# GSByeon/multi-speaker-tacotron-tensorflow

Measured on AMD Instinct MI355X. Metric: mel-frames/sec (batched decode), higher is better.
Workload: dtype f32 storage and accumulation; feed-forward GEMMs as 3-term split-bf16 MFMA (bf16x3), the attention memory layer as 6-term split-bf16 MFMA (operands split three ways: fp32-grade); recurrent / decoder mat-vecs exact fp32

## Files before the change

### multi-speaker-tacotron-tensorflow_amd/csrc/taco_decoder_xcd.h

```cpp
#pragma once
#include "taco_kernels.h"

typedef __attribute__((address_space(1))) unsigned long long dx_gu64;
typedef __attribute__((address_space(1))) unsigned dx_gu32;

#define DX_NT 512
#define DX_NW 8
#define DX_GROUP 32
#define DX_NGROUP 8
#define DX_W 256
#define DX_P2 128
#define DX_P3 64
#define DX_SPIN_LIMIT (1u << 21)
#ifndef DX_POLL_SLEEP
#define DX_POLL_SLEEP 0
#endif
#ifndef DX_FIRST_POLL_DELAY
#define DX_FIRST_POLL_DELAY 5
#endif
#ifndef DX_PRIO_OLD
#define DX_PRIO_OLD 1
#endif
#ifndef DX_POLL_DELAY_B
#define DX_POLL_DELAY_B 5
#endif
#define DX_TRACE_STEPS 8
#define DX_TRACE_SLOTS 16

enum {
  DXR_P2 = 0,
  DXR_AGH = 4,
  DXR_AGX = 12,
  DXR_AC = 18,
  DXR_G1H = 22,
  DXR_G1A = 30,
  DXR_G1B = 46,
  DXR_G1C = 62,
  DXR_G2H = 66,
  DXR_G2X = 74,
  DXR_G2C = 86,
  DXR_P1C = 90,
  DXR_P1O = 94,
  DXR_F = 98,
  DX_NREG = 106
};

enum { DXS_P2 = 0, DXS_HATT = 128, DXS_CTX = 384, DXS_OUT2 = 640, DXS_T = 896, DXS_H1 = 1152, DXS_OUT1 = 1408, DXS_H2 = 1664,
       DXS_LD = 1920 };
enum { DXB_P1 = 0, DXB_P2, DXB_AR, DXB_AU, DXB_AC, DXB_G1R, DXB_G1U, DXB_G1X, DXB_O0, DXB_G1C, DXB_G2R, DXB_G2U, DXB_G2C, DXB_F0, DXB_F1,
       DXB_P3, DXB_N };
enum { DXRB_AR = 0, DXRB_AU, DXRB_AX, DXRB_G1R, DXRB_G1U, DXRB_G1X, DXRB_O0, DXRB_N };

enum { DXT_P1 = 0, DXT_HA, DXT_RA, DXT_UA, DXT_CA, DXT_RHA, DXT_Q, DXT_O0, DXT_R1, DXT_U1, DXT_C1, DXT_RH1, DXT_H1, DXT_O1,
       DXT_R2, DXT_U2, DXT_C2, DXT_RH2, DXT_H2, DXT_O2, DXT_N };

struct DxX { int p1, p2, rha, ha, sc, ctx, rh1, h1, o1, rh2, h2, p3, fb, total; };
__host__ __device__ inline DxX dx_xlayout(int RG, int T_in) {
  DxX x; int o = 0;
  x.p1 = o; o += RG * DX_W;  x.p2 = o; o += RG * DX_P2; x.rha = o; o += RG * DX_W; x.ha = o; o += RG * DX_W;
  x.sc = o; o += DX_GROUP * T_in;
  x.ctx = o; o += RG * DX_W; x.rh1 = o; o += RG * DX_W; x.h1 = o; o += RG * DX_W; x.o1 = o; o += RG * DX_W;
  x.rh2 = o; o += RG * DX_W; x.h2 = o; o += RG * DX_W;
  x.p3 = o; o += RG * DX_P3;
  x.fb = o; o += RG * DX_P2;
  x.total = o;
  return x;
}
__host__ __device__ inline size_t dx_lds_floats(int RG, int T_in, bool teacher = false, int AW = DX_W) {
  const int Pr = DX_GROUP / RG, DC = DX_W / Pr, Tpad = (T_in + 3) & ~3;
  const int Pc = Pr < 8 ? Pr : 8, Pp = Pr / Pc, DS = AW / Pc, TS = (T_in + Pp - 1) / Pp;
  size_t n = 0;
  n += (size_t)RG * DXS_LD;
  n += (size_t)TS * DS;
  n += (size_t)T_in * DC;
  n += 4 * (size_t)Tpad;
  n += 3 * 64;
  n += (size_t)DX_NW * 64;
  n += (size_t)DXB_N * DX_NW;
  n += (size_t)DXRB_N * RG * DX_NW;
  n += (size_t)((T_in + 63) & ~63);
  if (teacher) n += (size_t)RG * DX_W;
  n += 64;
  return n;
}
__host__ __device__ inline int dx_score_blocks(int RG) { const int Pr = DX_GROUP / RG; return Pr < 8 ? Pr : 8; }
__host__ __device__ inline int dx_q_regs(int RG, int AW = DX_W) { return (AW / dx_score_blocks(RG)) / 2; }

struct DxArgs {
  const float* wpack;
  const float* qpack;
  const float* b_p1_0; const float* b_p1c; const float* b_p2;
  const float* b_p3;
  const float* b_ag; const float* b_ac;
  const float* b_g1f;
  const float* b_g1c; const float* b_g2g; const float* b_g2c;
  const float* b_f;
  const float* att_v; const float* att_b; const float* score_bias;
  const float* keys; const float* values;
  const float* h_att0; const float* h10; const float* h20;
  const float* manual;
  const float* rowbias;
  const float* teacher;
  const float* p1o_raw;
  int own_fb;
  float* tape; size_t tstride;
  float* tp_p2; float* tp_ctx; int ld_p2, ld_ctx;
  float* tp_e; float* tp_alpha;
  int mels;
  float* mel; float* hist; int* nz; float* dbg;
  unsigned long long* xbuf; unsigned* ctl; unsigned* err; long long* trace;
  int B, T_in, n, rM, att_type, grp0, ngroups, force_wt, dbgw;
  int trc_member, trc_tid;
};

#define DX_DPP0(v, ctrl) __int_as_float(__builtin_amdgcn_update_dpp(0, __float_as_int(v), (ctrl), 0xF, 0xF, false))
#define DX_DPPZ(v, ctrl, rmask, bmask) __int_as_float(__builtin_amdgcn_update_dpp(0, __float_as_int(v), (ctrl), (rmask), (bmask), true))
__device__ __forceinline__ float dx_allsum(float v) {
  v += DX_DPP0(v, 0xB1);
  v += DX_DPP0(v, 0x4E);
  v += DX_DPP0(v, 0x141);
  v += DX_DPP0(v, 0x140);
  v += DX_DPPZ(v, 0x142, 0xA, 0xF);
  v += DX_DPPZ(v, 0x143, 0xC, 0xF);
  return __int_as_float(__builtin_amdgcn_readlane(__float_as_int(v), 63));
}
__device__ __forceinline__ float dx_allmax(float v) {
  v = fmaxf(v, DX_DPP0(v, 0xB1)); v = fmaxf(v, DX_DPP0(v, 0x4E)); v = fmaxf(v, DX_DPP0(v, 0x141)); v = fmaxf(v, DX_DPP0(v, 0x140));
  const float a = __int_as_float(__builtin_amdgcn_readlane(__float_as_int(v), 0)), b = __int_as_float(__builtin_amdgcn_readlane(__float_as_int(v), 16));
  const float c = __int_as_float(__builtin_amdgcn_readlane(__float_as_int(v), 32)), d = __int_as_float(__builtin_amdgcn_readlane(__float_as_int(v), 48));
  return fmaxf(fmaxf(a, b), fmaxf(c, d));
}
__device__ __forceinline__ float dx_quadsum(float v) { v += DX_DPP0(v, 0xB1); v += DX_DPP0(v, 0x4E); return v; }
__device__ __forceinline__ float dx_scan(float v) {
  float t = v + DX_DPPZ(v, 0x111, 0xF, 0xF);
  t += DX_DPPZ(v, 0x112, 0xF, 0xF);
  t += DX_DPPZ(v, 0x113, 0xF, 0xF);
  t += DX_DPPZ(t, 0x114, 0xF, 0xE);
  t += DX_DPPZ(t, 0x118, 0xF, 0xC);
  t += DX_DPPZ(t, 0x142, 0xA, 0xF);
  t += DX_DPPZ(t, 0x143, 0xC, 0xF);
  return t;
}
__device__ __forceinline__ float dx_sigmoid_fast(float x) { return __builtin_amdgcn_rcpf(1.0f + __builtin_amdgcn_exp2f(-1.4426950408889634f * x)); }

template <int REG0, int NCOLS, int RG, int NW = DX_NREG, int LD = DXS_LD>
__device__ __forceinline__ void dx_pass(const float (&W)[NW], const float* x, int lane, float (&acc)[NCOLS][RG]) {
#pragma unroll
  for (int r = 0; r < RG; ++r) {
    const float4 xv = *reinterpret_cast<const float4*>(x + r * LD + 4 * lane);
#pragma unroll
    for (int c = 0; c < NCOLS; ++c) {
      acc[c][r] = fmaf(W[REG0 + 4 * c + 0], xv.x, acc[c][r]);
      acc[c][r] = fmaf(W[REG0 + 4 * c + 1], xv.y, acc[c][r]);
      acc[c][r] = fmaf(W[REG0 + 4 * c + 2], xv.z, acc[c][r]);
      acc[c][r] = fmaf(W[REG0 + 4 * c + 3], xv.w, acc[c][r]);
    }
  }
}
template <int REG0, int NCOLS, int RG>
__device__ __forceinline__ void dx_pass2(const float (&W)[DX_NREG], const float* x, int lane, float (&acc)[NCOLS][RG]) {
#pragma unroll
  for (int r = 0; r < RG; ++r) {
    const float2 xv = *reinterpret_cast<const float2*>(x + r * DXS_LD + 2 * lane);
#pragma unroll
    for (int c = 0; c < NCOLS; ++c) {
      acc[c][r] = fmaf(W[REG0 + 2 * c + 0], xv.x, acc[c][r]);
      acc[c][r] = fmaf(W[REG0 + 2 * c + 1], xv.y, acc[c][r]);
    }
  }
}
template <int REG0, int NCOLS, int RG>
__device__ __forceinline__ void dx_pass1(const float (&W)[DX_NREG], const float* x, int lane, float (&acc)[NCOLS][RG]) {
#pragma unroll
  for (int r = 0; r < RG; ++r) {
    const float xv = x[r * DXS_LD + lane];
#pragma unroll
    for (int c = 0; c < NCOLS; ++c) acc[c][r] = fmaf(W[REG0 + c], xv, acc[c][r]);
  }
}
template <int NCOLS, int RG>
__device__ __forceinline__ void dx_zero(float (&acc)[NCOLS][RG]) {
#pragma unroll
  for (int c = 0; c < NCOLS; ++c)
#pragma unroll
    for (int r = 0; r < RG; ++r) acc[c][r] = 0.f;
}
template <int RG> struct DxRL { static constexpr int value = RG >= 4 ? RG / 4 : 1; };
template <int RG>
__device__ __forceinline__ int dx_row(int lane, int q) {
  if (RG >= 4) return (lane & 1) * (RG / 2) + ((lane >> 1) & 1) * (RG / 4) + q;
  if (RG == 2) return lane & 1;
  return 0;
}
__device__ __forceinline__ float dx_xrow16(float v) {
  const unsigned u = __float_as_uint(v);
  auto r = __builtin_amdgcn_permlane16_swap(u, u, false, false);
  return __uint_as_float(r[0]) + __uint_as_float(r[1]);
}
__device__ __forceinline__ float dx_xrow32(float v) {
  const unsigned u = __float_as_uint(v);
  auto r = __builtin_amdgcn_permlane32_swap(u, u, false, false);
  return __uint_as_float(r[0]) + __uint_as_float(r[1]);
}
template <int NC, int RG>
__device__ __forceinline__ void dx_reduce(const float (&a)[NC][RG], float (&out)[NC][DxRL<RG>::value], int lane) {
  constexpr int RL = DxRL<RG>::value;
  const bool b0 = (lane & 1) != 0, b1 = (lane & 2) != 0;
  float d[NC][RL];
  if (RG >= 4) {
    constexpr int H = RG / 2, Q = RG / 4;
    float b[NC][H];
#pragma unroll
    for (int c = 0; c < NC; ++c)
#pragma unroll
      for (int p = 0; p < H; ++p) {
        const float keep = b0 ? a[c][H + p] : a[c][p], send = b0 ? a[c][p] : a[c][H + p];
        b[c][p] = keep + DX_DPP0(send, 0xB1);
      }
#pragma unroll
    for (int c = 0; c < NC; ++c)
#pragma unroll
      for (int q = 0; q < Q; ++q) {
        const float keep = b1 ? b[c][Q + q] : b[c][q], send = b1 ? b[c][q] : b[c][Q + q];
        d[c][q] = keep + DX_DPP0(send, 0x4E);
      }
  } else if (RG == 2) {
#pragma unroll
    for (int c = 0; c < NC; ++c) {
      const float keep = b0 ? a[c][1] : a[c][0], send = b0 ? a[c][0] : a[c][1];
      const float t = keep + DX_DPP0(send, 0xB1);
      d[c][0] = t + DX_DPP0(t, 0x4E);
    }
  } else {
#pragma unroll
    for (int c = 0; c < NC; ++c) {
      const float t = a[c][0] + DX_DPP0(a[c][0], 0xB1);
      d[c][0] = t + DX_DPP0(t, 0x4E);
    }
  }
#pragma unroll
  for (int c = 0; c < NC; ++c)
#pragma unroll
    for (int q = 0; q < RL; ++q) d[c][q] += DX_DPP0(d[c][q], 0x124);
#pragma unroll
  for (int c = 0; c < NC; ++c)
#pragma unroll
    for (int q = 0; q < RL; ++q) d[c][q] += DX_DPP0(d[c][q], 0x128);
#pragma unroll
  for (int c = 0; c < NC; ++c)
#pragma unroll
    for (int q = 0; q < RL; ++q) d[c][q] = dx_xrow16(d[c][q]);
#pragma unroll
  for (int c = 0; c < NC; ++c)
#pragma unroll
    for (int q = 0; q < RL; ++q) out[c][q] = dx_xrow32(d[c][q]);
}

#ifndef DX_DIET
#define DX_DIET 1
#endif
#define DX_NWP (DX_NREG / 2)
__host__ __device__ constexpr int dxw_two(int base, int r, int h) { return base + (r - base) / 2 + 4 * h; }
__host__ __device__ constexpr int dxw_src(int k, int h, int PD) {
  const int r = 2 * k;
  if (r >= DXR_AGH && r < DXR_AGX) return dxw_two(DXR_AGH, r, h);
  if (r >= DXR_AGX && r < DXR_AC) return PD == 3 ? r + h : (r < DXR_AGX + 4 ? DXR_AGX + (r - DXR_AGX) / 2 + 2 * h : r + h);
  if (r >= DXR_G1H && r < DXR_G1A) return dxw_two(DXR_G1H, r, h);
  if (r >= DXR_G1A && r < DXR_G1C) return dxw_two(DXR_G1A + 8 * ((r - DXR_G1A) / 8), r, h);
  if (r >= DXR_G2H && r < DXR_G2X) return dxw_two(DXR_G2H, r, h);
  if (r >= DXR_G2X && r < DXR_G2X + 8) return dxw_two(DXR_G2X, r, h);
  if (r >= DXR_F) return dxw_two(DXR_F, r, h);
  return r + h;
}
#define DXQ_FMA(acc, xs, wp) \
  do { if (DX_DIET) acc = __builtin_elementwise_fma((taco_f32x2){xs, xs}, wp, acc); else { acc.x = fmaf((wp).x, xs, acc.x); acc.y = fmaf((wp).y, xs, acc.y); } } while (0)
template <int RG>
__device__ __forceinline__ void dxq_zero(taco_f32x2 (&acc)[RG]) {
#pragma unroll
  for (int r = 0; r < RG; ++r) acc[r] = (taco_f32x2){0.f, 0.f};
}
template <int REG0, int RG, int LD = DXS_LD>
__device__ __forceinline__ void dxw_single(const taco_f32x2 (&WP)[DX_NWP], const float* x, int lane, float (&acc)[1][RG]) {
  constexpr int k = REG0 / 2;
#pragma unroll
  for (int r = 0; r < RG; ++r) {
    const float4 xv = *reinterpret_cast<const float4*>(x + r * LD + 4 * lane);
    acc[0][r] = fmaf(WP[k].x, xv.x, acc[0][r]); acc[0][r] = fmaf(WP[k].y, xv.y, acc[0][r]);
    acc[0][r] = fmaf(WP[k + 1].x, xv.z, acc[0][r]); acc[0][r] = fmaf(WP[k + 1].y, xv.w, acc[0][r]);
  }
}
template <int REG0, int RG, int LD = DXS_LD>
__device__ __forceinline__ void dxw_pair(const taco_f32x2 (&WP)[DX_NWP], const float* x, int lane, taco_f32x2 (&acc)[RG]) {
  constexpr int k = REG0 / 2;
#pragma unroll
  for (int r = 0; r < RG; ++r) {
    const float4 xv = *reinterpret_cast<const float4*>(x + r * LD + 4 * lane);
    DXQ_FMA(acc[r], xv.x, WP[k]); DXQ_FMA(acc[r], xv.y, WP[k + 1]); DXQ_FMA(acc[r], xv.z, WP[k + 2]); DXQ_FMA(acc[r], xv.w, WP[k + 3]);
  }
}
template <int REG0, int RG, int LD = DXS_LD>
__device__ __forceinline__ void dxw_quad(const taco_f32x2 (&WP)[DX_NWP], const float* x, int lane, taco_f32x2 (&p0)[RG], taco_f32x2 (&p1)[RG]) {
  constexpr int k = REG0 / 2;
#pragma unroll
  for (int r = 0; r < RG; ++r) {
    const float4 xv = *reinterpret_cast<const float4*>(x + r * LD + 4 * lane);
    DXQ_FMA(p0[r], xv.x, WP[k]); DXQ_FMA(p1[r], xv.x, WP[k + 4]);
    DXQ_FMA(p0[r], xv.y, WP[k + 1]); DXQ_FMA(p1[r], xv.y, WP[k + 5]);
    DXQ_FMA(p0[r], xv.z, WP[k + 2]); DXQ_FMA(p1[r], xv.z, WP[k + 6]);
    DXQ_FMA(p0[r], xv.w, WP[k + 3]); DXQ_FMA(p1[r], xv.w, WP[k + 7]);
  }
}
template <int REGP, int REGS, int RG, int LD = DXS_LD>
__device__ __forceinline__ void dxw_pair_single(const taco_f32x2 (&WP)[DX_NWP], const float* x, int lane, taco_f32x2 (&p)[RG], float (&sg)[1][RG]) {
  constexpr int k = REGP / 2, ks = REGS / 2;
#pragma unroll
  for (int r = 0; r < RG; ++r) {
    const float4 xv = *reinterpret_cast<const float4*>(x + r * LD + 4 * lane);
    DXQ_FMA(p[r], xv.x, WP[k]); sg[0][r] = fmaf(WP[ks].x, xv.x, sg[0][r]);
    DXQ_FMA(p[r], xv.y, WP[k + 1]); sg[0][r] = fmaf(WP[ks].y, xv.y, sg[0][r]);
    DXQ_FMA(p[r], xv.z, WP[k + 2]); sg[0][r] = fmaf(WP[ks + 1].x, xv.z, sg[0][r]);
    DXQ_FMA(p[r], xv.w, WP[k + 3]); sg[0][r] = fmaf(WP[ks + 1].y, xv.w, sg[0][r]);
  }
}
template <int RG>
__device__ __forceinline__ void dxw_agx2(const taco_f32x2 (&WP)[DX_NWP], const float* x, int lane, taco_f32x2 (&p)[RG], float (&sg)[1][RG]) {
  constexpr int k = DXR_AGX / 2;
#pragma unroll
  for (int r = 0; r < RG; ++r) {
    const float2 xv = *reinterpret_cast<const float2*>(x + r * DXS_LD + 2 * lane);
    DXQ_FMA(p[r], xv.x, WP[k]); sg[0][r] = fmaf(WP[k + 2].x, xv.x, sg[0][r]);
    DXQ_FMA(p[r], xv.y, WP[k + 1]); sg[0][r] = fmaf(WP[k + 2].y, xv.y, sg[0][r]);
  }
}
template <int RG>
__device__ __forceinline__ void dxw_agx1(const taco_f32x2 (&WP)[DX_NWP], const float* x, int lane, taco_f32x2 (&p)[RG], float (&sg)[1][RG]) {
  constexpr int k = DXR_AGX / 2;
#pragma unroll
  for (int r = 0; r < RG; ++r) {
    const float xv = x[r * DXS_LD + lane];
    DXQ_FMA(p[r], xv, WP[k]); sg[0][r] = fmaf(WP[k + 1].x, xv, sg[0][r]);
  }
}
template <int RG>
__device__ __forceinline__ void dxw_p3(const taco_f32x2 (&WP)[DX_NWP], const float* x, int lane, float (&acc)[1][RG]) {
  constexpr int k = DXR_AGX / 2;
#pragma unroll
  for (int r = 0; r < RG; ++r) {
    const float2 xv = *reinterpret_cast<const float2*>(x + r * DXS_LD + 2 * lane);
    acc[0][r] = fmaf(WP[k + 1].y, xv.x, acc[0][r]); acc[0][r] = fmaf(WP[k + 2].x, xv.y, acc[0][r]);
  }
}
template <int RG>
__device__ __forceinline__ int dxs_row(int lane, int q) {
  if (!DX_DIET) return dx_row<RG>(lane & 3, q);
  if (RG >= 8) return ((lane >> 4) & 1) * (RG / 4) + (lane >> 5) * (RG / 2) + q;
  if (RG == 4) return lane >> 4;
  if (RG == 2) return lane >> 5;
  return 0;
}
template <int RG>
__device__ __forceinline__ bool dxs_epl(int lane) {
  if (!DX_DIET) return lane < (RG >= 4 ? 4 : RG);
  return RG >= 4 ? (lane & 15) == 0 : RG == 2 ? (lane & 31) == 0 : lane == 0;
}
template <int NC, int RG>
__device__ __forceinline__ void dxs_reduce(const float (&a)[NC][RG], float (&out)[NC][DxRL<RG>::value], int lane) {
  if constexpr (!DX_DIET) { dx_reduce<NC, RG>(a, out, lane); return; }
  else {
    constexpr int RL = DxRL<RG>::value;
    float d[NC][RL];
    if constexpr (RG >= 4) {
      constexpr int Hh = RG / 2, Q = RG / 4;
      float b[NC][Hh];
#pragma unroll
      for (int c = 0; c < NC; ++c)
#pragma unroll
        for (int p = 0; p < Hh; ++p) {
          auto r = __builtin_amdgcn_permlane32_swap(__float_as_uint(a[c][p]), __float_as_uint(a[c][Hh + p]), false, false);
          b[c][p] = __uint_as_float(r[0]) + __uint_as_float(r[1]);
        }
#pragma unroll
      for (int c = 0; c < NC; ++c)
#pragma unroll
        for (int q = 0; q < Q; ++q) {
          auto r = __builtin_amdgcn_permlane16_swap(__float_as_uint(b[c][q]), __float_as_uint(b[c][Q + q]), false, false);
          d[c][q] = __uint_as_float(r[0]) + __uint_as_float(r[1]);
        }
    } else if constexpr (RG == 2) {
#pragma unroll
      for (int c = 0; c < NC; ++c) {
        auto r = __builtin_amdgcn_permlane32_swap(__float_as_uint(a[c][0]), __float_as_uint(a[c][1]), false, false);
        d[c][0] = dx_xrow16(__uint_as_float(r[0]) + __uint_as_float(r[1]));
      }
    } else {
#pragma unroll
      for (int c = 0; c < NC; ++c) d[c][0] = dx_xrow16(dx_xrow32(a[c][0]));
    }
#pragma unroll
    for (int c = 0; c < NC; ++c)
#pragma unroll
      for (int q = 0; q < RL; ++q) d[c][q] += DX_DPP0(d[c][q], 0xB1);
#pragma unroll
    for (int c = 0; c < NC; ++c)
#pragma unroll
      for (int q = 0; q < RL; ++q) d[c][q] += DX_DPP0(d[c][q], 0x4E);
#pragma unroll
    for (int c = 0; c < NC; ++c)
#pragma unroll
      for (int q = 0; q < RL; ++q) d[c][q] += DX_DPP0(d[c][q], 0x141);
#pragma unroll
    for (int c = 0; c < NC; ++c)
#pragma unroll
      for (int q = 0; q < RL; ++q) out[c][q] = d[c][q] + DX_DPP0(d[c][q], 0x140);
  }
}

#ifndef DX_DLY_TUNED
#define DX_DLY_TUNED 1
#endif
__host__ __device__ constexpr int dx_site_delay(int site, int dflt, int RG = 4) {
  constexpr int tuned4[11] = {4, 5, 6, 5, 0, 0, 5, 5, 0, 4, 0};
  constexpr int tuned8[11] = {7, 5, 3, 5, 0, 6, 5, 6, 4, 6, 2};
  return DX_DLY_TUNED ? (RG == 8 ? tuned8[site] : tuned4[site]) : dflt;
}
#ifdef DX_DLY_RT
__constant__ int g_dx_dly[32];
#define DX_DLY(site, dflt) (100 + (site))
#else
#define DX_DLY(site, dflt) dx_site_delay(site, dflt, RG)
#endif
struct DxRt {
  dx_gu32* err; bool wt; bool dead;
#ifdef DX_DLY_RT
  int dly[12];
#endif
};
template <int DLY>
__device__ __forceinline__ void dx_first_poll_sleep(const DxRt& rt) {
#ifdef DX_DLY_RT
  if constexpr (DLY >= 100) { const int n = __builtin_amdgcn_readfirstlane(rt.dly[DLY - 100]); for (int i = 0; i < n; ++i) __builtin_amdgcn_s_sleep(1); return; }
#endif
  if constexpr (DLY > 0 && DLY < 100) __builtin_amdgcn_s_sleep(DLY);
  (void)rt;
}
#ifndef DX_PUB_MODE
#define DX_PUB_MODE 0
#endif
__device__ __forceinline__ void dx_store_local(dx_gu64* p, unsigned long long g) {
  if (DX_PUB_MODE == 1) (void)__hip_atomic_exchange(p, g, __ATOMIC_RELAXED, __HIP_MEMORY_SCOPE_WORKGROUP);
  else if (DX_PUB_MODE == 2) __builtin_nontemporal_store(g, p);
  else if (DX_PUB_MODE == 3) *p = g;
  else __hip_atomic_store(p, g, __ATOMIC_RELAXED, __HIP_MEMORY_SCOPE_WORKGROUP);
}
template <int WTC = -1>
__device__ __forceinline__ void dx_publish(dx_gu64* p, float v, unsigned tag, const DxRt& rt) {
  const unsigned long long g = ((unsigned long long)tag << 32) | (unsigned long long)__float_as_uint(v);
  if (WTC == 1 || (WTC < 0 && rt.wt)) __hip_atomic_store(p, g, __ATOMIC_RELAXED, __HIP_MEMORY_SCOPE_AGENT);
  else dx_store_local(p, g);
}
template <int N, int WTC = -1>
__device__ __forceinline__ void dx_publish_n(dx_gu64* p, int stride, const float (&v)[N], unsigned tag, const DxRt& rt) {
  unsigned long long g[N];
#pragma unroll
  for (int u = 0; u < N; ++u) g[u] = ((unsigned long long)tag << 32) | (unsigned long long)__float_as_uint(v[u]);
  if (WTC == 1 || (WTC < 0 && rt.wt)) {
#pragma unroll
    for (int u = 0; u < N; ++u) __hip_atomic_store(p + u * stride, g[u], __ATOMIC_RELAXED, __HIP_MEMORY_SCOPE_AGENT);
  } else {
#pragma unroll
    for (int u = 0; u < N; ++u) dx_store_local(p + u * stride, g[u]);
  }
}
#define DX_PIN(x) asm("" : "+v"(x))
template <int N, int DLY = 0>
__device__ __forceinline__ void dx_poll(const dx_gu64* p0, size_t stride, unsigned tag, float (&v)[N], DxRt& rt) {
  unsigned long long g[N];
  unsigned spins = 0;
  dx_first_poll_sleep<DLY>(rt);
  for (;;) {
    bool ok = true;
#pragma unroll
    for (int u = 0; u < N; ++u) g[u] = __hip_atomic_load(p0 + u * stride, __ATOMIC_RELAXED, __HIP_MEMORY_SCOPE_AGENT);
#pragma unroll
    for (int u = 0; u < N; ++u) ok = ok && ((unsigned)(g[u] >> 32) == tag);
    if (ok || rt.dead) break;
    if (DX_POLL_SLEEP) __builtin_amdgcn_s_sleep(DX_POLL_SLEEP);
    if ((++spins & 1023u) == 0) {
      if (spins >= DX_SPIN_LIMIT || __hip_atomic_load(rt.err, __ATOMIC_RELAXED, __HIP_MEMORY_SCOPE_AGENT) != 0) {
        __hip_atomic_store(rt.err, 2u, __ATOMIC_RELAXED, __HIP_MEMORY_SCOPE_AGENT);
        rt.dead = true;
      }
    }
  }
#pragma unroll
  for (int u = 0; u < N; ++u) v[u] = __uint_as_float((unsigned)g[u]);
}
typedef unsigned long long dx_u64x2 __attribute__((ext_vector_type(2)));
template <int NP, int DLY = 0>
__device__ __forceinline__ void dx_poll_pairs(const dx_gu64* p0, size_t stride, unsigned tag, float (&v)[2 * NP], DxRt& rt) {
  dx_u64x2 g[NP];
  unsigned spins = 0;
  dx_first_poll_sleep<DLY>(rt);
  for (;;) {
    bool ok = true;
#pragma unroll
    for (int u = 0; u < NP; ++u) {
      const dx_gu64* p = p0 + u * stride;
      asm volatile("global_load_dwordx4 %0, %1, off sc1" : "=v"(g[u]) : "v"(p) : "memory");
    }
    asm volatile("s_waitcnt vmcnt(0)" ::: "memory");
#pragma unroll
    for (int u = 0; u < NP; ++u) ok = ok && ((unsigned)(g[u][0] >> 32) == tag) && ((unsigned)(g[u][1] >> 32) == tag);
    if (ok || rt.dead) break;
    if ((++spins & 1023u) == 0) {
      if (spins >= DX_SPIN_LIMIT || __hip_atomic_load(rt.err, __ATOMIC_RELAXED, __HIP_MEMORY_SCOPE_AGENT) != 0) {
        __hip_atomic_store(rt.err, 2u, __ATOMIC_RELAXED, __HIP_MEMORY_SCOPE_AGENT);
        rt.dead = true;
      }
    }
  }
#pragma unroll
  for (int u = 0; u < NP; ++u) { v[2 * u] = __uint_as_float((unsigned)g[u][0]); v[2 * u + 1] = __uint_as_float((unsigned)g[u][1]); }
}
template <int RG, int N, bool RES, int LD = DXS_LD, int NT = DX_NT, int DLY = 0>
__device__ __forceinline__ void dx_gather(const dx_gu64* X, unsigned tag, float* st, int off, int off_res, int off2, int tid, DxRt& rt) {
  constexpr int NI = (RG * N + NT - 1) / NT;
  if constexpr (NI >= 4 && NI % 2 == 0 && (RG * N) % (2 * NT) == 0 && N % 2 == 0) {
    constexpr int NP = NI / 2;
    float v[NI];
    dx_poll_pairs<NP, DLY>(X + 2 * tid, (size_t)2 * NT, tag, v, rt);
#pragma unroll
    for (int u = 0; u < NP; ++u) {
      const int i = 2 * (u * NT + tid), r = i / N, n = i % N;
      *reinterpret_cast<float2*>(st + r * LD + off + n) = make_float2(v[2 * u], v[2 * u + 1]);
      if (RES) {
        const float2 rs = *reinterpret_cast<const float2*>(st + r * LD + off_res + n);
        *reinterpret_cast<float2*>(st + r * LD + off2 + n) = make_float2(v[2 * u] + rs.x, v[2 * u + 1] + rs.y);
      }
    }
    return;
  }
  const bool act = (RG * N >= NT) || tid < RG * N;
  if (act) {
    float v[NI];
    dx_poll<NI, DLY>(X + tid, NT, tag, v, rt);
#pragma unroll
    for (int u = 0; u < NI; ++u) {
      const int i = u * NT + tid;
      const int r = i / N, n = i % N;
      st[r * LD + off + n] = v[u];
      if (RES) st[r * LD + off2 + n] = v[u] + st[r * LD + off_res + n];
    }
  }
}

template <int CMAX>
__device__ __forceinline__ void dx_normalise(float* sc, const float* alp, int j0, int cnt, int att_type, float sbias) {
  float e[CMAX], pv[CMAX];
#pragma unroll
  for (int i = 0; i < CMAX; ++i) { e[i] = i < cnt ? sc[j0 + i] : 0.f; pv[i] = i < cnt ? alp[j0 + i] : 0.f; }
  if (att_type == 2) {
    float p[CMAX], ex[CMAX], run = 0.f;
#pragma unroll
    for (int i = 0; i < CMAX; ++i) {
      p[i] = dx_sigmoid_fast(e[i] + sbias);
      ex[i] = run;
      if (i < cnt) run += 0.6931471805599453f * __builtin_amdgcn_logf(fminf(fmaxf(1.f - p[i], 1.17549435e-38f), 1.f));
    }
    const float off = dx_scan(run) - run;
    float cp[CMAX], in2[CMAX], run2 = 0.f;
#pragma unroll
    for (int i = 0; i < CMAX; ++i) {
      cp[i] = __builtin_amdgcn_exp2f(1.4426950408889634f * (ex[i] + off));
      if (i < cnt) run2 += pv[i] * __builtin_amdgcn_rcpf(fminf(fmaxf(cp[i], 1e-10f), 1.f));
      in2[i] = run2;
    }
    const float off2 = dx_scan(run2) - run2;
#pragma unroll
    for (int i = 0; i < CMAX; ++i) if (i < cnt) sc[j0 + i] = p[i] * cp[i] * (in2[i] + off2);
  } else {
    float mx = -INFINITY;
#pragma unroll
    for (int i = 0; i < CMAX; ++i) if (i < cnt) mx = fmaxf(mx, e[i]);
    mx = dx_allmax(mx);
    float sm = 0.f;
#pragma unroll
    for (int i = 0; i < CMAX; ++i) { e[i] = __builtin_amdgcn_exp2f(1.4426950408889634f * (e[i] - mx)); if (i < cnt) sm += e[i]; }
    sm = dx_allsum(sm);
    const float inv = 1.0f / sm;
#pragma unroll
    for (int i = 0; i < CMAX; ++i) if (i < cnt) sc[j0 + i] = e[i] * inv;
  }
}
__device__ __forceinline__ void dx_normalise_lds(float* sc, float* tmp, float* tmp2, const float* alp, int j0, int j1, int att_type, float sbias) {
  if (att_type == 2) {
    float run = 0.f;
    for (int j = j0; j < j1; ++j) {
      const float p = dx_sigmoid_fast(sc[j] + sbias);
      const float lg = 0.6931471805599453f * __builtin_amdgcn_logf(fminf(fmaxf(1.f - p, 1.17549435e-38f), 1.f));
      sc[j] = p; tmp[j] = run; run += lg;
    }
    const float off = dx_scan(run) - run;
    float run2 = 0.f;
    for (int j = j0; j < j1; ++j) {
      const float cp = __builtin_amdgcn_exp2f(1.4426950408889634f * (tmp[j] + off));
      tmp[j] = cp;
      run2 += alp[j] * __builtin_amdgcn_rcpf(fminf(fmaxf(cp, 1e-10f), 1.f));
      tmp2[j] = run2;
    }
    const float off2 = dx_scan(run2) - run2;
    for (int j = j0; j < j1; ++j) sc[j] = sc[j] * tmp[j] * (tmp2[j] + off2);
  } else {
    float mx = -INFINITY;
    for (int j = j0; j < j1; ++j) mx = fmaxf(mx, sc[j]);
    mx = dx_allmax(mx);
    float sm = 0.f;
    for (int j = j0; j < j1; ++j) { const float e = __builtin_amdgcn_exp2f(1.4426950408889634f * (sc[j] - mx)); sc[j] = e; sm += e; }
    sm = dx_allsum(sm);
    const float inv = 1.0f / sm;
    for (int j = j0; j < j1; ++j) sc[j] = sc[j] * inv;
  }
}

typedef __attribute__((address_space(3))) float dx_lds_float;
__device__ __forceinline__ void dx_load_lds4(const float* gsrc, unsigned lds_dst) {
  unsigned keep;
  asm volatile("s_mov_b32 %0, m0\n\ts_mov_b32 m0, %2\n\ts_nop 0\n\tglobal_load_lds_dword %1, off\n\ts_mov_b32 m0, %0"
               : "=&s"(keep) : "v"(gsrc), "s"(lds_dst) : "memory");
}

__device__ __forceinline__ void dx_census(dx_gu32* ctl, dx_gu32* errw, int force_wt, int* out, int tid, int info0) {
  if (tid == 0) {
    const unsigned xcc = __builtin_amdgcn_s_getreg(6164) & 7u;
    const unsigned slot = __hip_atomic_fetch_add(ctl + xcc, 1u, __ATOMIC_RELAXED, __HIP_MEMORY_SCOPE_AGENT);
    __hip_atomic_fetch_add(ctl + 8, 1u, __ATOMIC_RELAXED, __HIP_MEMORY_SCOPE_AGENT);
    unsigned spins = 0; bool ok = true;
    while (__hip_atomic_load(ctl + 8, __ATOMIC_RELAXED, __HIP_MEMORY_SCOPE_AGENT) < gridDim.x) {
      __builtin_amdgcn_s_sleep(2);
      if (++spins > (DX_SPIN_LIMIT << 2) || __hip_atomic_load(errw, __ATOMIC_RELAXED, __HIP_MEMORY_SCOPE_AGENT) != 0) { ok = false; break; }
    }
    bool even = ok;
    for (int i = 0; i < DX_NGROUP; ++i)
      even = even && (__hip_atomic_load(ctl + i, __ATOMIC_RELAXED, __HIP_MEMORY_SCOPE_AGENT) == gridDim.x / DX_NGROUP);
    const bool fast = even && !force_wt;
    if (!ok) __hip_atomic_store(errw, 1u, __ATOMIC_RELAXED, __HIP_MEMORY_SCOPE_AGENT);
    out[0] = fast ? (int)xcc : (int)(blockIdx.x & 7);
    out[1] = fast ? (int)slot : (int)(blockIdx.x >> 3);
    out[2] = fast ? 0 : 1;
    out[3] = ok ? 0 : 1;
    if (blockIdx.x == 0) {
      errw[info0] = fast ? 1u : 2u;
      for (int i = 0; i < DX_NGROUP; ++i) errw[info0 + 1 + i] = __hip_atomic_load(ctl + i, __ATOMIC_RELAXED, __HIP_MEMORY_SCOPE_AGENT);
    }
  }
  __syncthreads();
}

__global__ __launch_bounds__(DX_W) void k_dx_rowbias(const float* table, const int* speaker_id, const float* spkw, int S, float* rowbias) {
  const int b = blockIdx.x, n = threadIdx.x;
  const float* e = table + (size_t)(speaker_id ? speaker_id[b] : b) * S;
  for (int slot = 0; slot < DXRB_N; ++slot) {
    float acc = 0.f;
    for (int k = 0; k < S; ++k) acc = fmaf(e[k], spkw[((size_t)k * DXRB_N + slot) * DX_W + n], acc);
    rowbias[((size_t)b * DXRB_N + slot) * DX_W + n] = acc;
  }
}

#define DX_STAMP(slot)                                                                                     \
  do {                                                                                                     \
    if constexpr (TRACE) { if (tracer && t < DX_TRACE_STEPS) a.trace[t * DX_TRACE_SLOTS + (slot)] = (long long)__builtin_readcyclecounter(); } \
  } while (0)

template <int RG, bool TAPE, bool MAN, int AW, int PD, bool WT, bool TRACE>
__device__ __forceinline__ void dx_body(const DxArgs& a, float* dx_smem, int group, int member, DxRt rt) {
  static_assert((AW == DX_W && PD == 2) || !TAPE, "the training forward exists at the reference widths only");
  constexpr int WTC = WT ? 1 : 0;
  const int tid = threadIdx.x, lane = tid & 63;
  const int wave = __builtin_amdgcn_readfirstlane(tid >> 6);
  constexpr int Pr = DX_GROUP / RG;
  constexpr int DC = DX_W / Pr;
  constexpr int Pc = Pr < 8 ? Pr : 8, Pp = Pr / Pc;
  constexpr int DS = AW / Pc;
  static_assert(DS >= 8 && DS <= 64, "query columns per wave / the qv, vv, bq slots");
  constexpr int QC = DS / 8;
  constexpr int QR = 4 * QC;
  constexpr int CH = DS / 4;
  constexpr int NP = Pc / 4;
  const int T = a.T_in, Tpad = (T + 3) & ~3;
  const int TP = (T + Pr - 1) / Pr;
  const int TS = (T + Pp - 1) / Pp;

  float* st = dx_smem;
  float* Kc = st + RG * DXS_LD;
  float* Vc = Kc + (size_t)TS * DS;
  float* sc = Vc + (size_t)T * DC;
  float* tmp = sc + Tpad;
  float* tmp2 = tmp + Tpad;
  float* alp = tmp2 + Tpad;
  float* qv = alp + Tpad;
  float* vv = qv + 64;
  float* bq = vv + 64;
  float* cpart = bq + 64;
  float* bl = cpart + DX_NW * 64;
  float* rbl = bl + DXB_N * DX_NW;
  float* mrow = rbl + DXRB_N * RG * DX_NW;
  float* tfb = mrow + ((T + 63) & ~63);
  const int ga = (group - a.grp0) & 7;
  if (ga >= a.ngroups || member >= DX_GROUP) return;
  const int row0 = ga * RG;
  if (row0 >= a.B) return;
  const int arow = member / Pr, asl = member % Pr;
  const int cb = asl % Pc, pb = asl / Pc;
  const int ps0 = pb * TS, psn = max(0, min(T - ps0, TS));
  const int brow = row0 + arow;
  const bool tracer = TRACE && a.trace && ga == 0 && member == a.trc_member && tid == a.trc_tid;

  taco_f32x2 WP[DX_NWP];
  {
    const float* wp = a.wpack + ((size_t)member * DX_NREG) * DX_NT + tid;
#pragma unroll
    for (int k = 0; k < DX_NWP; ++k) WP[k] = (taco_f32x2){wp[(size_t)dxw_src(k, 0, PD) * DX_NT], wp[(size_t)dxw_src(k, 1, PD) * DX_NT]};
  }
  if (TAPE && a.p1o_raw) {
    const float* wp = a.p1o_raw + ((size_t)member * 4) * DX_NT + tid;
    WP[DXR_P1O / 2] = (taco_f32x2){wp[0], wp[(size_t)DX_NT]};
    WP[DXR_P1O / 2 + 1] = (taco_f32x2){wp[(size_t)2 * DX_NT], wp[(size_t)3 * DX_NT]};
  }
  taco_f32x2 WQP[QR / 2];
  {
    const float* wp = a.qpack + ((size_t)member * QR) * DX_NT + tid;
#pragma unroll
    for (int j = 0; j < QC / 2; ++j)
#pragma unroll
      for (int e = 0; e < 4; ++e) WQP[4 * j + e] = (taco_f32x2){wp[(size_t)(8 * j + e) * DX_NT], wp[(size_t)(8 * j + 4 + e) * DX_NT]};
  }
  const DxX xl = dx_xlayout(RG, T);
  dx_gu64* X = (dx_gu64*)a.xbuf + (size_t)ga * xl.total;
  const int NCF = (a.rM + DX_GROUP - 1) / DX_GROUP;

  for (int i = tid; i < TS * (DS / 4); i += DX_NT) {
    const int j = i / (DS / 4), d4 = i % (DS / 4);
    float4 k4 = make_float4(0.f, 0.f, 0.f, 0.f);
    if (brow < a.B && j < psn) k4 = *reinterpret_cast<const float4*>(a.keys + ((size_t)brow * T + ps0 + j) * AW + cb * DS + 4 * d4);
    *reinterpret_cast<float4*>(Kc + (size_t)j * DS + 4 * d4) = k4;
  }
  for (int i = tid; i < T * (DC / 4); i += DX_NT) {
    const int j = i / (DC / 4), d4 = i % (DC / 4);
    float4 v4 = make_float4(0.f, 0.f, 0.f, 0.f);
    if (brow < a.B) v4 = *reinterpret_cast<const float4*>(a.values + ((size_t)brow * T + j) * DX_W + asl * DC + 4 * d4);
    *reinterpret_cast<float4*>(Vc + (size_t)j * DC + 4 * d4) = v4;
  }
  for (int i = tid; i < RG * DXS_LD; i += DX_NT) st[i] = 0.f;
  __syncthreads();
  for (int i = tid; i < RG * DX_W; i += DX_NT) {
    const int r = i / DX_W, nn = i % DX_W, b = row0 + r;
    if (b < a.B) {
      if (a.h_att0) st[r * DXS_LD + DXS_HATT + nn] = a.h_att0[(size_t)b * DX_W + nn];
      if (a.h10) st[r * DXS_LD + DXS_H1 + nn] = a.h10[(size_t)b * DX_W + nn];
      if (a.h20) st[r * DXS_LD + DXS_H2 + nn] = a.h20[(size_t)b * DX_W + nn];
    }
    st[r * DXS_LD + DXS_T + nn] = fmaxf(a.b_p1_0[nn], 0.f);
  }
  for (int j = tid; j < Tpad; j += DX_NT) { alp[j] = (a.att_type == 2 && j == 0) ? 1.f : 0.f; sc[j] = 0.f; tmp[j] = 0.f; tmp2[j] = 0.f; }
  if (tid < DS) { vv[tid] = a.att_v[cb * DS + tid]; bq[tid] = a.att_b ? a.att_b[cb * DS + tid] : 0.f; qv[tid] = 0.f; }
  if (tid < DXB_N * DX_NW) {
    const int e = tid / DX_NW, w = tid % DX_NW, n8 = member * 8 + w;
    float v = 0.f;
    switch (e) {
      case DXB_P1: v = (TAPE && a.p1o_raw) ? a.b_p1_0[n8] : a.b_p1c[n8]; break;
      case DXB_P2: if (w < 4) v = a.b_p2[member * 4 + w]; break;
      case DXB_AR: v = a.b_ag[n8]; break;
      case DXB_AU: v = a.b_ag[DX_W + n8]; break;
      case DXB_AC: v = a.b_ac[n8]; break;
      case DXB_G1R: v = a.b_g1f[n8]; break;
      case DXB_G1U: v = a.b_g1f[DX_W + n8]; break;
      case DXB_G1X: v = a.b_g1f[2 * DX_W + n8]; break;
      case DXB_O0: v = a.b_g1f[3 * DX_W + n8]; break;
      case DXB_G1C: v = a.b_g1c[n8]; break;
      case DXB_G2R: v = a.b_g2g[n8]; break;
      case DXB_G2U: v = a.b_g2g[DX_W + n8]; break;
      case DXB_G2C: v = a.b_g2c[n8]; break;
      case DXB_F0: if (w < NCF && member * NCF + w < a.rM) v = a.b_f[member * NCF + w]; break;
      case DXB_F1: if (w + 8 < NCF && member * NCF + w + 8 < a.rM) v = a.b_f[member * NCF + w + 8]; break;
      case DXB_P3: if (PD == 3 && w < 2) v = a.b_p3[member * 2 + w]; break;
      default: break;
    }
    bl[tid] = v;
  }
  for (int i = tid; i < DXRB_N * RG * DX_NW; i += DX_NT) {
    const int e = i / (RG * DX_NW), r = (i / DX_NW) % RG, w = i % DX_NW, b = row0 + r, n8 = member * 8 + w;
    float v = 0.f;
    switch (e) {
      case DXRB_AR: v = a.b_ag[n8]; break;
      case DXRB_AU: v = a.b_ag[DX_W + n8]; break;
      case DXRB_AX: v = 0.f; break;
      case DXRB_G1R: v = a.b_g1f[n8]; break;
      case DXRB_G1U: v = a.b_g1f[DX_W + n8]; break;
      case DXRB_G1X: v = a.b_g1f[2 * DX_W + n8]; break;
      default: v = a.b_g1f[3 * DX_W + n8]; break;
    }
    if (a.rowbias && b < a.B) v += a.rowbias[((size_t)b * DXRB_N + e) * DX_W + n8];
    rbl[i] = v;
  }
  const float sbias = (a.att_type == 2 && a.score_bias) ? a.score_bias[0] : 0.f;
  constexpr bool man = MAN;
  const unsigned mrow_lds = (unsigned)(size_t)(dx_lds_float*)mrow;
  const unsigned tfb_lds = (unsigned)(size_t)(dx_lds_float*)tfb;
  if (TAPE) for (int i = tid; i < RG * DX_W; i += DX_NT) tfb[i] = 0.f;
  __syncthreads();

  constexpr int RL = DxRL<RG>::value;
  const bool epl = dxs_epl<RG>(lane);
  const int en = member * 8 + wave;
  int erow[RL];
#pragma unroll
  for (int q = 0; q < RL; ++q) erow[q] = dxs_row<RG>(lane, q);
#define DX_RB(slot, q) rbl[((slot) * RG + erow[q]) * DX_NW + wave]
  float g_u[RL], g_cx[RL], g_h[RL], g_o0[RL];
  unsigned trow[RL];
  bool tval[RL];
  float g_o1[RL];
  const unsigned tstr = (unsigned)a.tstride;
#pragma unroll
  for (int q = 0; q < RL; ++q) {
    trow[q] = (unsigned)(row0 + erow[q]) * (unsigned)a.n * DX_W + (unsigned)en;
    tval[q] = TAPE && a.tape && epl && (row0 + erow[q] < a.B);
    g_o1[q] = 0.f;
  }
#define DX_TAPE(slot, q, val) do { if (TAPE && tval[q]) a.tape[(unsigned)(slot) * tstr + trow[q] + (unsigned)t * DX_W] = (val); } while (0)
  if (TAPE) {
    const int t = 0;
#pragma unroll
    for (int q = 0; q < RL; ++q) DX_TAPE(DXT_P1, q, fmaxf(a.b_p1_0[en], 0.f));
  }

  if (DX_PRIO_OLD && wave < 4) __builtin_amdgcn_s_setprio(DX_PRIO_OLD);
  const int tid_outer = tid, lane_outer = lane;
  for (int t = 0; t < a.n; ++t) {
    const unsigned tag = (unsigned)t + 1u;
    int tid = tid_outer, lane = lane_outer;
    asm volatile("" : "+v"(tid), "+v"(lane));
    int erow[RL];
#pragma unroll
    for (int q = 0; q < RL; ++q) erow[q] = dxs_row<RG>(lane, q);
    DX_STAMP(0);
    if (man) {
      const float* src = a.manual + ((size_t)min(brow, a.B - 1) * a.n + t) * T;
      for (int j0 = wave * 64; j0 < T; j0 += DX_NT)
        dx_load_lds4(src + min(j0 + lane, T - 1), __builtin_amdgcn_readfirstlane(mrow_lds + (unsigned)j0 * 4u));
    }
    if (TAPE && a.teacher && wave < RG && t + 1 < a.n) {
      const float* src = a.teacher + ((size_t)min(row0 + wave, a.B - 1) * a.n + t) * a.mels;
      for (int j0 = 0; j0 < a.mels; j0 += 64)
        dx_load_lds4(src + min(j0 + lane, a.mels - 1), __builtin_amdgcn_readfirstlane(tfb_lds + (unsigned)(wave * DX_W + j0) * 4u));
    }
    if (wave < 4) {
      float acc[1][RG], s[1][RL];
      dx_zero<1, RG>(acc);
      dxw_single<DXR_P2, RG>(WP, st + DXS_T, lane, acc);
      dxs_reduce<1, RG>(acc, s, lane);
      if (epl) {
#pragma unroll
        for (int q = 0; q < RL; ++q) {
          const float p2v = fmaxf(s[0][q] + bl[DXB_P2 * DX_NW + wave], 0.f);
          dx_publish<WTC>(X + xl.p2 + erow[q] * DX_P2 + member * 4 + wave, p2v, tag, rt);
          if (TAPE && tval[q] && a.tp_p2) a.tp_p2[((size_t)(row0 + erow[q]) * a.n + t) * a.ld_p2 + member * 4 + wave] = p2v;
        }
      }
    }
#pragma unroll
    for (int q = 0; q < RL; ++q) g_h[q] = st[erow[q] * DXS_LD + DXS_HATT + en];
    taco_f32x2 ag01[RG];
    float ag2[1][RG];
    dxq_zero<RG>(ag01);
    dx_zero<1, RG>(ag2);
    dxw_pair<DXR_AGH, RG>(WP, st + DXS_HATT, lane, ag01);
    dx_gather<RG, DX_P2, false, DXS_LD, DX_NT, DX_DLY(0, DX_POLL_DELAY_B)>(X + xl.p2, tag, st, DXS_P2, 0, 0, tid, rt);
    __syncthreads();
    if constexpr (PD == 3) {
      if (wave < 2) {
        float acc[1][RG], s[1][RL];
        dx_zero<1, RG>(acc);
        dxw_p3<RG>(WP, st + DXS_P2, lane, acc);
        dxs_reduce<1, RG>(acc, s, lane);
        if (epl) {
#pragma unroll
          for (int q = 0; q < RL; ++q)
            dx_publish<WTC>(X + xl.p3 + erow[q] * DX_P3 + member * 2 + wave, fmaxf(s[0][q] + bl[DXB_P3 * DX_NW + wave], 0.f), tag, rt);
        }
      }
      dx_gather<RG, DX_P3, false, DXS_LD, DX_NT, DX_DLY(1, DX_FIRST_POLL_DELAY)>(X + xl.p3, tag, st, DXS_OUT2, 0, 0, tid, rt);
      __syncthreads();
    }
    DX_STAMP(1);
    {
      float s[3][RL];
      if constexpr (PD == 3) dxw_agx1<RG>(WP, st + DXS_OUT2, lane, ag01, ag2);
      else dxw_agx2<RG>(WP, st + DXS_P2, lane, ag01, ag2);
      float aga[3][RG];
#pragma unroll
      for (int r = 0; r < RG; ++r) { aga[0][r] = ag01[r].x; aga[1][r] = ag01[r].y; aga[2][r] = ag2[0][r]; }
      dxs_reduce<3, RG>(aga, s, lane);
#pragma unroll
      for (int q = 0; q < RL; ++q) {
        const float rg = dx_sigmoid_fast(s[0][q] + DX_RB(DXRB_AR, q));
        g_u[q] = dx_sigmoid_fast(s[1][q] + DX_RB(DXRB_AU, q));
        g_cx[q] = s[2][q] + DX_RB(DXRB_AX, q);
        if (epl) dx_publish<WTC>(X + xl.rha + erow[q] * DX_W + en, rg * g_h[q], tag, rt);
        DX_TAPE(DXT_RA, q, rg); DX_TAPE(DXT_UA, q, g_u[q]); DX_TAPE(DXT_RHA, q, rg * g_h[q]);
      }
    }
    dx_gather<RG, DX_W, false, DXS_LD, DX_NT, DX_DLY(2, DX_FIRST_POLL_DELAY)>(X + xl.rha, tag, st, DXS_T, 0, 0, tid, rt);
    __syncthreads();
    DX_STAMP(2);
    {
      float acc[1][RG], s[1][RL];
      dx_zero<1, RG>(acc);
      dxw_single<DXR_AC, RG>(WP, st + DXS_T, lane, acc);
      dxs_reduce<1, RG>(acc, s, lane);
#pragma unroll
      for (int q = 0; q < RL; ++q) {
        const float c = taco_tanh_fast(g_cx[q] + s[0][q] + bl[DXB_AC * DX_NW + wave]);
        const float hn = g_u[q] * g_h[q] + (1.f - g_u[q]) * c;
        if (epl) dx_publish<WTC>(X + xl.ha + erow[q] * DX_W + en, hn, tag, rt);
        DX_TAPE(DXT_CA, q, c); DX_TAPE(DXT_HA, q, hn);
      }
    }
#pragma unroll
    for (int q = 0; q < RL; ++q) g_h[q] = st[erow[q] * DXS_LD + DXS_H1 + en];
    dx_gather<RG, DX_W, false, DXS_LD, DX_NT, DX_DLY(3, DX_FIRST_POLL_DELAY)>(X + xl.ha, tag, st, DXS_HATT, 0, 0, tid, rt);
    __syncthreads();
    DX_STAMP(3);
    if (!man) {
      {
        const float4 xv = *reinterpret_cast<const float4*>(st + arow * DXS_LD + DXS_HATT + 4 * lane);
        float qa[QC][1], qs[QC][1];
        static_assert(QC % 2 == 0, "query columns in pairs");
#pragma unroll
        for (int i = 0; i < QC; i += 2) {
          taco_f32x2 q2 = {0.f, 0.f};
          DXQ_FMA(q2, xv.x, WQP[2 * i + 0]); DXQ_FMA(q2, xv.y, WQP[2 * i + 1]); DXQ_FMA(q2, xv.z, WQP[2 * i + 2]); DXQ_FMA(q2, xv.w, WQP[2 * i + 3]);
          qa[i][0] = q2.x; qa[i + 1][0] = q2.y;
        }
        dxs_reduce<QC, 1>(qa, qs, lane);
        float qme = qs[0][0];
#pragma unroll
        for (int i = 1; i < QC; ++i) qme = (lane >= i) ? qs[i][0] : qme;
        if (lane < QC) qv[wave * QC + lane] = qme + bq[wave * QC + lane];
        if (TAPE && a.tape && lane < QC && pb == 0 && brow < a.B)
          a.tape[(unsigned)DXT_Q * tstr + ((unsigned)brow * (unsigned)a.n + (unsigned)t) * DX_W + cb * DS + wave * QC + lane] = qme;
      }
      __syncthreads();
      DX_STAMP(4);
      {
        const int jl = lane >> 2, cp = lane & 3;
        constexpr bool QV_REG = CH < 16;
        float qreg[QV_REG ? CH : 1], vreg[QV_REG ? CH : 1];
        if constexpr (QV_REG) {
#pragma unroll
          for (int c = 0; c < CH; ++c) { qreg[c] = qv[cp * CH + c]; vreg[c] = vv[cp * CH + c]; }
        }
        for (int j0 = 0; j0 < psn; j0 += 16 * DX_NW) {
          const int j = j0 + wave * 16 + jl;
          const int jc = j < psn ? j : psn - 1;
          const float* kp = Kc + (size_t)jc * DS + cp * CH;
          float e = 0.f;
#pragma unroll
          for (int c = 0; c < CH; c += 4) {
            const float4 k4 = *reinterpret_cast<const float4*>(kp + c);
            if constexpr (QV_REG) {
              e += vreg[c] * taco_tanh_fast(k4.x + qreg[c]) + vreg[c + 1] * taco_tanh_fast(k4.y + qreg[c + 1]) +
                   vreg[c + 2] * taco_tanh_fast(k4.z + qreg[c + 2]) + vreg[c + 3] * taco_tanh_fast(k4.w + qreg[c + 3]);
            } else {
              const float4 q4 = *reinterpret_cast<const float4*>(qv + cp * CH + c), v4 = *reinterpret_cast<const float4*>(vv + cp * CH + c);
              e += v4.x * taco_tanh_fast(k4.x + q4.x) + v4.y * taco_tanh_fast(k4.y + q4.y) +
                   v4.z * taco_tanh_fast(k4.z + q4.z) + v4.w * taco_tanh_fast(k4.w + q4.w);
            }
          }
          e = dx_quadsum(e);
          if (cp == 0 && j < psn) dx_publish<WTC>(X + xl.sc + (size_t)(arow * Pc + cb) * T + ps0 + j, e, tag, rt);
        }
      }
    }
    constexpr bool G1_AHEAD = RG < 8;
    taco_f32x2 g1p0[RG], g1p1[RG];
    dxq_zero<RG>(g1p0); dxq_zero<RG>(g1p1);
    if (G1_AHEAD) {
      dxw_pair<DXR_G1H, RG>(WP, st + DXS_H1, lane, g1p0);
      dxw_quad<DXR_G1A, RG>(WP, st + DXS_HATT, lane, g1p0, g1p1);
    }
    int aoff = 0;
    if (!man) {
      {
        const int jl = lane >> 2, part = lane & 3;
        for (int j0 = 0; j0 < T; j0 += 16 * DX_NW) {
          const int j = j0 + wave * 16 + jl;
          float s = 0.f;
          if (j < T) {
            float v[NP];
            dx_poll<NP, DX_DLY(4, DX_POLL_DELAY_B)>(X + xl.sc + (size_t)(arow * Pc + part * NP) * T + j, (size_t)T, tag, v, rt);
#pragma unroll
            for (int u = 0; u < NP; ++u) s += v[u];
          }
          s = dx_quadsum(s);
          if (part == 0 && j < T) sc[j] = s;
        }
      }
      __syncthreads();
      DX_STAMP(5);
      if (TAPE && a.tp_e && tid < TP && asl * TP + tid < T && brow < a.B)
        a.tp_e[((size_t)brow * a.n + t) * T + asl * TP + tid] = sc[asl * TP + tid];
      if (TAPE) __syncthreads();
      if (wave == 0) {
        const int C = (T + 63) >> 6;
        const int j0 = lane * C;
        if (C <= 2) dx_normalise<2>(sc, alp, j0, min(C, max(T - j0, 0)), a.att_type, sbias);
        else if (C <= 8) dx_normalise<8>(sc, alp, j0, min(C, max(T - j0, 0)), a.att_type, sbias);
        else dx_normalise_lds(sc, tmp, tmp2, alp, j0, min(j0 + C, T), a.att_type, sbias);
      }
      __syncthreads();
    } else {
      asm volatile("s_waitcnt vmcnt(0)" ::: "memory");
      __syncthreads();
      aoff = (int)(mrow - sc);
    }
    {
      for (int j = tid; j < T; j += DX_NT) alp[j] = sc[aoff + j];
      const int p0 = asl * TP;
      if (tid < TP && p0 + tid < T && brow < a.B) {
        if (a.hist) a.hist[((size_t)brow * T + p0 + tid) * a.n + t] = sc[aoff + p0 + tid];
        if (TAPE && a.tp_alpha) a.tp_alpha[((size_t)brow * (a.n + 1) + t + 1) * T + p0 + tid] = sc[aoff + p0 + tid];
      }
      constexpr int JL = 64 / DC;
      const int d = lane % DC, jsub = lane / DC;
      float part = 0.f;
      for (int j = wave * JL + jsub; j < T; j += DX_NW * JL) part = fmaf(sc[aoff + j], Vc[(size_t)j * DC + d], part);
      if (DC <= 32) part = dx_xrow32(part);
      if (DC <= 16) part = dx_xrow16(part);
      if (DC <= 8) part += DX_DPP0(part, 0x128);
      if (lane < DC) cpart[wave * 64 + lane] = part;
    }
    __syncthreads();
    if (tid < DC) {
      float s = 0.f;
#pragma unroll
      for (int w = 0; w < DX_NW; ++w) s += cpart[w * 64 + tid];
      dx_publish<WTC>(X + xl.ctx + arow * DX_W + asl * DC + tid, s, tag, rt);
      if (TAPE && a.tp_ctx && brow < a.B) a.tp_ctx[((size_t)brow * a.n + t) * a.ld_ctx + asl * DC + tid] = s;
    }
    dx_gather<RG, DX_W, false, DXS_LD, DX_NT, DX_DLY(5, DX_FIRST_POLL_DELAY)>(X + xl.ctx, tag, st, DXS_CTX, 0, 0, tid, rt);
    __syncthreads();
    DX_STAMP(6);
    {
      float s[4][RL];
      if (!G1_AHEAD) {
        dxq_zero<RG>(g1p0); dxq_zero<RG>(g1p1);
        dxw_pair<DXR_G1H, RG>(WP, st + DXS_H1, lane, g1p0);
        dxw_quad<DXR_G1A, RG>(WP, st + DXS_HATT, lane, g1p0, g1p1);
      }
      dxw_quad<DXR_G1B, RG>(WP, st + DXS_CTX, lane, g1p0, g1p1);
      float g1a[4][RG];
#pragma unroll
      for (int r = 0; r < RG; ++r) { g1a[0][r] = g1p0[r].x; g1a[1][r] = g1p0[r].y; g1a[2][r] = g1p1[r].x; g1a[3][r] = g1p1[r].y; }
      dxs_reduce<4, RG>(g1a, s, lane);
      DX_STAMP(12);
#pragma unroll
      for (int q = 0; q < RL; ++q) {
        const float rg = dx_sigmoid_fast(s[0][q] + DX_RB(DXRB_G1R, q));
        g_u[q] = dx_sigmoid_fast(s[1][q] + DX_RB(DXRB_G1U, q));
        g_cx[q] = s[2][q] + DX_RB(DXRB_G1X, q);
        g_o0[q] = s[3][q] + DX_RB(DXRB_O0, q);
        if (epl) dx_publish<WTC>(X + xl.rh1 + erow[q] * DX_W + en, rg * g_h[q], tag, rt);
        DX_TAPE(DXT_R1, q, rg); DX_TAPE(DXT_U1, q, g_u[q]); DX_TAPE(DXT_RH1, q, rg * g_h[q]); DX_TAPE(DXT_O0, q, g_o0[q]);
      }
      DX_STAMP(13);
    }
    dx_gather<RG, DX_W, false, DXS_LD, DX_NT, DX_DLY(6, DX_FIRST_POLL_DELAY)>(X + xl.rh1, tag, st, DXS_T, 0, 0, tid, rt);
    DX_STAMP(14);
    __syncthreads();
    DX_STAMP(7);
    {
      float acc[1][RG], s[1][RL];
      dx_zero<1, RG>(acc);
      dxw_single<DXR_G1C, RG>(WP, st + DXS_T, lane, acc);
      dxs_reduce<1, RG>(acc, s, lane);
#pragma unroll
      for (int q = 0; q < RL; ++q) {
        const float c = taco_tanh_fast(g_cx[q] + s[0][q] + bl[DXB_G1C * DX_NW + wave]);
        const float hn = g_u[q] * g_h[q] + (1.f - g_u[q]) * c;
        g_o1[q] = hn + g_o0[q];
        if (epl) {
          dx_publish<WTC>(X + xl.h1 + erow[q] * DX_W + en, hn, tag, rt);
          dx_publish<WTC>(X + xl.o1 + erow[q] * DX_W + en, hn + g_o0[q], tag, rt);
        }
        DX_TAPE(DXT_C1, q, c); DX_TAPE(DXT_H1, q, hn); DX_TAPE(DXT_O1, q, g_o1[q]);
      }
    }
#pragma unroll
    for (int q = 0; q < RL; ++q) g_h[q] = st[erow[q] * DXS_LD + DXS_H2 + en];
    taco_f32x2 g2p[RG];
    float g2c[1][RG];
    dxq_zero<RG>(g2p);
    dx_zero<1, RG>(g2c);
    if (G1_AHEAD) dxw_pair<DXR_G2H, RG>(WP, st + DXS_H2, lane, g2p);
    dx_gather<RG, DX_W, false, DXS_LD, DX_NT, DX_DLY(7, DX_POLL_DELAY_B)>(X + xl.h1, tag, st, DXS_H1, 0, 0, tid, rt);
    dx_gather<RG, DX_W, false, DXS_LD, DX_NT, 0>(X + xl.o1, tag, st, DXS_OUT1, 0, 0, tid, rt);
    __syncthreads();
    DX_STAMP(8);
    {
      float s[3][RL];
      if (!G1_AHEAD) dxw_pair<DXR_G2H, RG>(WP, st + DXS_H2, lane, g2p);
      dxw_pair_single<DXR_G2X, DXR_G2X + 8, RG>(WP, st + DXS_OUT1, lane, g2p, g2c);
      float g2a[3][RG];
#pragma unroll
      for (int r = 0; r < RG; ++r) { g2a[0][r] = g2p[r].x; g2a[1][r] = g2p[r].y; g2a[2][r] = g2c[0][r]; }
      dxs_reduce<3, RG>(g2a, s, lane);
#pragma unroll
      for (int q = 0; q < RL; ++q) {
        const float rg = dx_sigmoid_fast(s[0][q] + bl[DXB_G2R * DX_NW + wave]);
        g_u[q] = dx_sigmoid_fast(s[1][q] + bl[DXB_G2U * DX_NW + wave]);
        g_cx[q] = s[2][q];
        if (epl) dx_publish<WTC>(X + xl.rh2 + erow[q] * DX_W + en, rg * g_h[q], tag, rt);
        DX_TAPE(DXT_R2, q, rg); DX_TAPE(DXT_U2, q, g_u[q]); DX_TAPE(DXT_RH2, q, rg * g_h[q]);
      }
    }
    dx_gather<RG, DX_W, false, DXS_LD, DX_NT, DX_DLY(8, DX_FIRST_POLL_DELAY)>(X + xl.rh2, tag, st, DXS_T, 0, 0, tid, rt);
    __syncthreads();
    DX_STAMP(9);
    {
      float acc[1][RG], s[1][RL];
      dx_zero<1, RG>(acc);
      dxw_single<DXR_G2C, RG>(WP, st + DXS_T, lane, acc);
      dxs_reduce<1, RG>(acc, s, lane);
#pragma unroll
      for (int q = 0; q < RL; ++q) {
        const float c = taco_tanh_fast(g_cx[q] + s[0][q] + bl[DXB_G2C * DX_NW + wave]);
        const float hn = g_u[q] * g_h[q] + (1.f - g_u[q]) * c;
        if (epl) dx_publish<WTC>(X + xl.h2 + erow[q] * DX_W + en, hn, tag, rt);
        DX_TAPE(DXT_C2, q, c); DX_TAPE(DXT_H2, q, hn); DX_TAPE(DXT_O2, q, hn + g_o1[q]);
      }
    }
    float p1a[1][RG];
    dx_zero<1, RG>(p1a);
    if (G1_AHEAD) dxw_single<DXR_P1C, RG>(WP, st + DXS_CTX, lane, p1a);
    dx_gather<RG, DX_W, true, DXS_LD, DX_NT, DX_DLY(9, DX_POLL_DELAY_B)>(X + xl.h2, tag, st, DXS_H2, DXS_OUT1, DXS_OUT2, tid, rt);
    __syncthreads();
    DX_STAMP(10);
    auto store_frame = [&](int q, float y0, float y1, bool share) {
      const int b = row0 + erow[q];
      const int n0 = member * NCF + wave, n1 = n0 + 8;
      const bool v0 = wave < NCF && n0 < a.rM, v1 = wave + 8 < NCF && n1 < a.rM;
      if (b < a.B) {
        float* mrow = a.mel + (size_t)b * a.n * a.rM + (size_t)t * a.rM;
        bool nzf = false;
        if (v0) { mrow[n0] = y0; nzf = nzf || (y0 != 0.f); }
        if (v1) { mrow[n1] = y1; nzf = nzf || (y1 != 0.f); }
        if (nzf) a.nz[(size_t)t * a.B + b] = 1;
      }
      if (share) {
        const int f0 = a.rM - a.mels;
        if (v0 && n0 >= f0) dx_publish<WTC>(X + xl.fb + erow[q] * DX_P2 + (n0 - f0), y0, tag, rt);
        if (v1 && n1 >= f0) dx_publish<WTC>(X + xl.fb + erow[q] * DX_P2 + (n1 - f0), y1, tag, rt);
      }
    };
    if (TAPE && a.own_fb) {
      {
        taco_f32x2 fp[RG];
        float fa[2][RG], s[2][RL];
        dxq_zero<RG>(fp);
        dxw_pair<DXR_F, RG>(WP, st + DXS_OUT2, lane, fp);
#pragma unroll
        for (int r = 0; r < RG; ++r) { fa[0][r] = fp[r].x; fa[1][r] = fp[r].y; }
        dxs_reduce<2, RG>(fa, s, lane);
        if (epl) {
#pragma unroll
          for (int q = 0; q < RL; ++q) store_frame(q, s[0][q] + bl[DXB_F0 * DX_NW + wave], s[1][q] + bl[DXB_F1 * DX_NW + wave], t + 1 < a.n);
        }
      }
      if (t + 1 < a.n) {
        for (int i = tid; i < RG * a.mels; i += DX_NT) {
          const int r = i / a.mels, j = i - r * a.mels;
          float v[1];
          dx_poll<1>(X + xl.fb + r * DX_P2 + j, 0, tag, v, rt);
          tfb[r * DX_W + j] = v[0];
        }
      }
      __syncthreads();
      {
        float pa[1][RG], s[1][RL];
#pragma unroll
        for (int r = 0; r < RG; ++r) pa[0][r] = p1a[0][r];
        if (!G1_AHEAD) dxw_single<DXR_P1C, RG>(WP, st + DXS_CTX, lane, pa);
        dxw_single<DXR_P1O, RG, DX_W>(WP, tfb, lane, pa);
        dxs_reduce<1, RG>(pa, s, lane);
        if (epl && t + 1 < a.n) {
#pragma unroll
          for (int q = 0; q < RL; ++q) {
            const float p1v = fmaxf(s[0][q] + bl[DXB_P1 * DX_NW + wave], 0.f);
            dx_publish<WTC>(X + xl.p1 + erow[q] * DX_W + en, p1v, tag, rt);
            if (tval[q]) a.tape[(unsigned)DXT_P1 * tstr + trow[q] + (unsigned)(t + 1) * DX_W] = p1v;
          }
        }
      }
    } else {
      taco_f32x2 fp[RG];
      float f2[1][RG], fa[3][RG], s[3][RL];
      dxq_zero<RG>(fp);
#pragma unroll
      for (int r = 0; r < RG; ++r) f2[0][r] = p1a[0][r];
      if (!G1_AHEAD) dxw_single<DXR_P1C, RG>(WP, st + DXS_CTX, lane, f2);
      if (TAPE) { dxw_pair<DXR_F, RG>(WP, st + DXS_OUT2, lane, fp); dxw_single<DXR_P1O, RG, DX_W>(WP, tfb, lane, f2); }
      else dxw_pair_single<DXR_F, DXR_P1O, RG>(WP, st + DXS_OUT2, lane, fp, f2);
#pragma unroll
      for (int r = 0; r < RG; ++r) { fa[0][r] = fp[r].x; fa[1][r] = fp[r].y; fa[2][r] = f2[0][r]; }
      dxs_reduce<3, RG>(fa, s, lane);
      if (epl) {
#pragma unroll
        for (int q = 0; q < RL; ++q) {
          if (t + 1 < a.n) {
            const float p1v = fmaxf(s[2][q] + bl[DXB_P1 * DX_NW + wave], 0.f);
            dx_publish<WTC>(X + xl.p1 + erow[q] * DX_W + en, p1v, tag, rt);
            if (TAPE && tval[q]) a.tape[(unsigned)DXT_P1 * tstr + trow[q] + (unsigned)(t + 1) * DX_W] = p1v;
          }
          store_frame(q, s[0][q] + bl[DXB_F0 * DX_NW + wave], s[1][q] + bl[DXB_F1 * DX_NW + wave], false);
        }
      }
    }
    if (a.dbg && member == 0) {
      for (int i = tid; i < RG * 4 * DX_W; i += DX_NT) {
        const int r = i / (4 * DX_W), q = (i / DX_W) & 3, nn = i % DX_W, b = row0 + r;
        const int off = q == 0 ? DXS_HATT : q == 1 ? DXS_CTX : q == 2 ? DXS_H1 : DXS_H2;
        if (b < a.B) a.dbg[((size_t)t * a.B + b) * a.dbgw + q * DX_W + nn] = st[r * DXS_LD + off + nn];
      }
    }
    if (t + 1 < a.n) dx_gather<RG, DX_W, false, DXS_LD, DX_NT, DX_DLY(10, DX_FIRST_POLL_DELAY)>(X + xl.p1, tag, st, DXS_T, 0, 0, tid, rt);
    __syncthreads();
    DX_STAMP(11);
  }
}

template <int RG, bool TAPE = false, bool MAN = false, int AW = DX_W, int PD = 2, bool TRACE = false>
__global__ __launch_bounds__(DX_NT) void k_decoder_xcd(const DxArgs a_in) {
  extern __shared__ __attribute__((aligned(16))) float dx_smem[];
  DxArgs a = a_in;
  int* ictl = reinterpret_cast<int*>(dx_smem + dx_lds_floats(RG, a.T_in, TAPE, AW) - 64);
  dx_gu32* errw = (dx_gu32*)a.err;
  dx_census((dx_gu32*)a.ctl, errw, a.force_wt, ictl, threadIdx.x, 8);
  const int group = __builtin_amdgcn_readfirstlane(ictl[0]);
  const int member = __builtin_amdgcn_readfirstlane(ictl[1]);
  DxRt rt; rt.err = errw; rt.wt = ictl[2] != 0; rt.dead = ictl[3] != 0;
#ifdef DX_DLY_RT
  { const int half = __builtin_amdgcn_readfirstlane((int)(threadIdx.x >> 8)) * 16; for (int i = 0; i < 12; ++i) rt.dly[i] = g_dx_dly[half + i]; }
#endif
  if (__builtin_amdgcn_readfirstlane((int)rt.wt)) dx_body<RG, TAPE, MAN, AW, PD, true, TRACE>(a, dx_smem, group, member, rt);
  else dx_body<RG, TAPE, MAN, AW, PD, false, TRACE>(a, dx_smem, group, member, rt);
}
```

Before: 6.180 million.

## Pin schedule across poll barriers, hoist bias loads, use 32-bit exchange addressing

Adds empty inline-asm register pins so partial mat-vec accumulators and bias loads are forced to finish before the spin-poll gathers, and batches LDS row loads ahead of the FMA loops. Moves alpha/history stores after the context publish so the cross-workgroup publish happens earlier. Replaces 64-bit pointer arithmetic on the exchange buffer with 32-bit index offsets to cut address VALU work in the poll and publish paths. Compiler scheduling is now constrained by the asm barriers, which may raise register pressure.

```diff
diff --git a/multi-speaker-tacotron-tensorflow_amd/csrc/taco_decoder_xcd.h b/multi-speaker-tacotron-tensorflow_amd/csrc/taco_decoder_xcd.h
--- a/multi-speaker-tacotron-tensorflow_amd/csrc/taco_decoder_xcd.h
+++ b/multi-speaker-tacotron-tensorflow_amd/csrc/taco_decoder_xcd.h
@@ -256,6 +256,17 @@
     for (int q = 0; q < RL; ++q) out[c][q] = dx_xrow32(d[c][q]);
 }
 
+template <int RG>
+__device__ __forceinline__ void dx_ahead(taco_f32x2 (&a)[RG]) {
+#pragma unroll
+  for (int r = 0; r < RG; ++r) asm volatile("" : "+v"(a[r]) : : "memory");
+}
+template <int RG>
+__device__ __forceinline__ void dx_ahead(float (&a)[1][RG]) {
+#pragma unroll
+  for (int r = 0; r < RG; ++r) asm volatile("" : "+v"(a[0][r]) : : "memory");
+}
+
 #ifndef DX_DIET
 #define DX_DIET 1
 #endif
@@ -272,6 +283,17 @@
   if (r >= DXR_F) return dxw_two(DXR_F, r, h);
   return r + h;
 }
+typedef float dx_f32x4 __attribute__((ext_vector_type(4)));
+template <int RG, int LD>
+__device__ __forceinline__ void dx_rows4(const float* x, int lane, dx_f32x4 (&xv)[RG]) {
+#pragma unroll
+  for (int r = 0; r < RG; ++r) xv[r] = *reinterpret_cast<const dx_f32x4*>(x + r * LD + 4 * lane);
+#pragma unroll
+  for (int r0 = 0; r0 < RG; r0 += 4) {
+    if constexpr (RG >= 4) asm volatile("" : "+v"(xv[r0]), "+v"(xv[r0 + 1]), "+v"(xv[r0 + 2]), "+v"(xv[r0 + 3]));
+    else if constexpr (RG == 2) asm volatile("" : "+v"(xv[0]), "+v"(xv[1]));
+  }
+}
 #define DXQ_FMA(acc, xs, wp) \
   do { if (DX_DIET) acc = __builtin_elementwise_fma((taco_f32x2){xs, xs}, wp, acc); else { acc.x = fmaf((wp).x, xs, acc.x); acc.y = fmaf((wp).y, xs, acc.y); } } while (0)
 template <int RG>
@@ -282,9 +304,11 @@
 template <int REG0, int RG, int LD = DXS_LD>
 __device__ __forceinline__ void dxw_single(const taco_f32x2 (&WP)[DX_NWP], const float* x, int lane, float (&acc)[1][RG]) {
   constexpr int k = REG0 / 2;
+  dx_f32x4 xr[RG];
+  dx_rows4<RG, LD>(x, lane, xr);
 #pragma unroll
   for (int r = 0; r < RG; ++r) {
-    const float4 xv = *reinterpret_cast<const float4*>(x + r * LD + 4 * lane);
+    const dx_f32x4 xv = xr[r];
     acc[0][r] = fmaf(WP[k].x, xv.x, acc[0][r]); acc[0][r] = fmaf(WP[k].y, xv.y, acc[0][r]);
     acc[0][r] = fmaf(WP[k + 1].x, xv.z, acc[0][r]); acc[0][r] = fmaf(WP[k + 1].y, xv.w, acc[0][r]);
   }
@@ -292,18 +316,22 @@
 template <int REG0, int RG, int LD = DXS_LD>
 __device__ __forceinline__ void dxw_pair(const taco_f32x2 (&WP)[DX_NWP], const float* x, int lane, taco_f32x2 (&acc)[RG]) {
   constexpr int k = REG0 / 2;
+  dx_f32x4 xr[RG];
+  dx_rows4<RG, LD>(x, lane, xr);
 #pragma unroll
   for (int r = 0; r < RG; ++r) {
-    const float4 xv = *reinterpret_cast<const float4*>(x + r * LD + 4 * lane);
+    const dx_f32x4 xv = xr[r];
     DXQ_FMA(acc[r], xv.x, WP[k]); DXQ_FMA(acc[r], xv.y, WP[k + 1]); DXQ_FMA(acc[r], xv.z, WP[k + 2]); DXQ_FMA(acc[r], xv.w, WP[k + 3]);
   }
 }
 template <int REG0, int RG, int LD = DXS_LD>
 __device__ __forceinline__ void dxw_quad(const taco_f32x2 (&WP)[DX_NWP], const float* x, int lane, taco_f32x2 (&p0)[RG], taco_f32x2 (&p1)[RG]) {
   constexpr int k = REG0 / 2;
+  dx_f32x4 xr[RG];
+  dx_rows4<RG, LD>(x, lane, xr);
 #pragma unroll
   for (int r = 0; r < RG; ++r) {
-    const float4 xv = *reinterpret_cast<const float4*>(x + r * LD + 4 * lane);
+    const dx_f32x4 xv = xr[r];
     DXQ_FMA(p0[r], xv.x, WP[k]); DXQ_FMA(p1[r], xv.x, WP[k + 4]);
     DXQ_FMA(p0[r], xv.y, WP[k + 1]); DXQ_FMA(p1[r], xv.y, WP[k + 5]);
     DXQ_FMA(p0[r], xv.z, WP[k + 2]); DXQ_FMA(p1[r], xv.z, WP[k + 6]);
@@ -313,9 +341,11 @@
 template <int REGP, int REGS, int RG, int LD = DXS_LD>
 __device__ __forceinline__ void dxw_pair_single(const taco_f32x2 (&WP)[DX_NWP], const float* x, int lane, taco_f32x2 (&p)[RG], float (&sg)[1][RG]) {
   constexpr int k = REGP / 2, ks = REGS / 2;
+  dx_f32x4 xr[RG];
+  dx_rows4<RG, LD>(x, lane, xr);
 #pragma unroll
   for (int r = 0; r < RG; ++r) {
-    const float4 xv = *reinterpret_cast<const float4*>(x + r * LD + 4 * lane);
+    const dx_f32x4 xv = xr[r];
     DXQ_FMA(p[r], xv.x, WP[k]); sg[0][r] = fmaf(WP[ks].x, xv.x, sg[0][r]);
     DXQ_FMA(p[r], xv.y, WP[k + 1]); sg[0][r] = fmaf(WP[ks].y, xv.y, sg[0][r]);
     DXQ_FMA(p[r], xv.z, WP[k + 2]); sg[0][r] = fmaf(WP[ks + 1].x, xv.z, sg[0][r]);
@@ -411,7 +441,10 @@
 #pragma unroll
     for (int c = 0; c < NC; ++c)
 #pragma unroll
-      for (int q = 0; q < RL; ++q) out[c][q] = d[c][q] + DX_DPP0(d[c][q], 0x140);
+      for (int q = 0; q < RL; ++q) {
+        out[c][q] = d[c][q] + DX_DPP0(d[c][q], 0x140);
+        asm("" : "+v"(out[c][q]));
+      }
   }
 }
 
@@ -452,6 +485,9 @@
   else if (DX_PUB_MODE == 3) *p = g;
   else __hip_atomic_store(p, g, __ATOMIC_RELAXED, __HIP_MEMORY_SCOPE_WORKGROUP);
 }
+__device__ __forceinline__ dx_gu64* dx_at(const dx_gu64* X, unsigned idx) {
+  return (dx_gu64*)((__attribute__((address_space(1))) char*)X + (size_t)(idx * 8u));
+}
 template <int WTC = -1>
 __device__ __forceinline__ void dx_publish(dx_gu64* p, float v, unsigned tag, const DxRt& rt) {
   const unsigned long long g = ((unsigned long long)tag << 32) | (unsigned long long)__float_as_uint(v);
@@ -473,14 +509,14 @@
 }
 #define DX_PIN(x) asm("" : "+v"(x))
 template <int N, int DLY = 0>
-__device__ __forceinline__ void dx_poll(const dx_gu64* p0, size_t stride, unsigned tag, float (&v)[N], DxRt& rt) {
+__device__ __forceinline__ void dx_poll_at(const dx_gu64* X, unsigned idx0, unsigned stride, unsigned tag, float (&v)[N], DxRt& rt) {
   unsigned long long g[N];
   unsigned spins = 0;
   dx_first_poll_sleep<DLY>(rt);
   for (;;) {
     bool ok = true;
 #pragma unroll
-    for (int u = 0; u < N; ++u) g[u] = __hip_atomic_load(p0 + u * stride, __ATOMIC_RELAXED, __HIP_MEMORY_SCOPE_AGENT);
+    for (int u = 0; u < N; ++u) g[u] = __hip_atomic_load(dx_at(X, idx0 + (unsigned)u * stride), __ATOMIC_RELAXED, __HIP_MEMORY_SCOPE_AGENT);
 #pragma unroll
     for (int u = 0; u < N; ++u) ok = ok && ((unsigned)(g[u] >> 32) == tag);
     if (ok || rt.dead) break;
@@ -495,9 +531,13 @@
 #pragma unroll
   for (int u = 0; u < N; ++u) v[u] = __uint_as_float((unsigned)g[u]);
 }
+template <int N, int DLY = 0>
+__device__ __forceinline__ void dx_poll(const dx_gu64* p0, size_t stride, unsigned tag, float (&v)[N], DxRt& rt) {
+  dx_poll_at<N, DLY>(p0, 0u, (unsigned)stride, tag, v, rt);
+}
 typedef unsigned long long dx_u64x2 __attribute__((ext_vector_type(2)));
 template <int NP, int DLY = 0>
-__device__ __forceinline__ void dx_poll_pairs(const dx_gu64* p0, size_t stride, unsigned tag, float (&v)[2 * NP], DxRt& rt) {
+__device__ __forceinline__ void dx_poll_pairs(const dx_gu64* X, unsigned idx0, unsigned stride, unsigned tag, float (&v)[2 * NP], DxRt& rt) {
   dx_u64x2 g[NP];
   unsigned spins = 0;
   dx_first_poll_sleep<DLY>(rt);
@@ -505,7 +545,7 @@
     bool ok = true;
 #pragma unroll
     for (int u = 0; u < NP; ++u) {
-      const dx_gu64* p = p0 + u * stride;
+      const dx_gu64* p = dx_at(X, idx0 + (unsigned)u * stride);
       asm volatile("global_load_dwordx4 %0, %1, off sc1" : "=v"(g[u]) : "v"(p) : "memory");
     }
     asm volatile("s_waitcnt vmcnt(0)" ::: "memory");
@@ -523,15 +563,15 @@
   for (int u = 0; u < NP; ++u) { v[2 * u] = __uint_as_float((unsigned)g[u][0]); v[2 * u + 1] = __uint_as_float((unsigned)g[u][1]); }
 }
 template <int RG, int N, bool RES, int LD = DXS_LD, int NT = DX_NT, int DLY = 0>
-__device__ __forceinline__ void dx_gather(const dx_gu64* X, unsigned tag, float* st, int off, int off_res, int off2, int tid, DxRt& rt) {
+__device__ __forceinline__ void dx_gather_at(const dx_gu64* X, unsigned base, unsigned tag, float* st, int off, int off_res, int off2, int tid, DxRt& rt) {
   constexpr int NI = (RG * N + NT - 1) / NT;
   if constexpr (NI >= 4 && NI % 2 == 0 && (RG * N) % (2 * NT) == 0 && N % 2 == 0) {
     constexpr int NP = NI / 2;
     float v[NI];
-    dx_poll_pairs<NP, DLY>(X + 2 * tid, (size_t)2 * NT, tag, v, rt);
+    dx_poll_pairs<NP, DLY>(X, base + 2u * (unsigned)tid, 2u * NT, tag, v, rt);
 #pragma unroll
     for (int u = 0; u < NP; ++u) {
-      const int i = 2 * (u * NT + tid), r = i / N, n = i % N;
+      const unsigned i = 2u * ((unsigned)(u * NT) + (unsigned)tid), r = i / (unsigned)N, n = i % (unsigned)N;
       *reinterpret_cast<float2*>(st + r * LD + off + n) = make_float2(v[2 * u], v[2 * u + 1]);
       if (RES) {
         const float2 rs = *reinterpret_cast<const float2*>(st + r * LD + off_res + n);
@@ -543,15 +583,19 @@
   const bool act = (RG * N >= NT) || tid < RG * N;
   if (act) {
     float v[NI];
-    dx_poll<NI, DLY>(X + tid, NT, tag, v, rt);
+    dx_poll_at<NI, DLY>(X, base + (unsigned)tid, NT, tag, v, rt);
 #pragma unroll
     for (int u = 0; u < NI; ++u) {
-      const int i = u * NT + tid;
-      const int r = i / N, n = i % N;
+      const unsigned i = (unsigned)(u * NT) + (unsigned)tid;
+      const unsigned r = i / (unsigned)N, n = i % (unsigned)N;
       st[r * LD + off + n] = v[u];
       if (RES) st[r * LD + off2 + n] = v[u] + st[r * LD + off_res + n];
     }
   }
+}
+template <int RG, int N, bool RES, int LD = DXS_LD, int NT = DX_NT, int DLY = 0>
+__device__ __forceinline__ void dx_gather(const dx_gu64* X, unsigned tag, float* st, int off, int off_res, int off2, int tid, DxRt& rt) {
+  dx_gather_at<RG, N, RES, LD, NT, DLY>(X, 0u, tag, st, off, off_res, off2, tid, rt);
 }
 
 template <int CMAX>
@@ -816,6 +860,8 @@
 #pragma unroll
   for (int q = 0; q < RL; ++q) erow[q] = dxs_row<RG>(lane, q);
 #define DX_RB(slot, q) rbl[((slot) * RG + erow[q]) * DX_NW + wave]
+#define DX_BIAS_AHEAD(var, slot) float var = bl[(slot) * DX_NW + wave]
+#define DX_BIAS_HERE(var) asm volatile("" : "+v"(var))
   float g_u[RL], g_cx[RL], g_h[RL], g_o0[RL];
   unsigned trow[RL];
   bool tval[RL];
@@ -856,14 +902,16 @@
     }
     if (wave < 4) {
       float acc[1][RG], s[1][RL];
+      DX_BIAS_AHEAD(b_p2, DXB_P2);
       dx_zero<1, RG>(acc);
       dxw_single<DXR_P2, RG>(WP, st + DXS_T, lane, acc);
+      DX_BIAS_HERE(b_p2);
       dxs_reduce<1, RG>(acc, s, lane);
       if (epl) {
 #pragma unroll
         for (int q = 0; q < RL; ++q) {
-          const float p2v = fmaxf(s[0][q] + bl[DXB_P2 * DX_NW + wave], 0.f);
-          dx_publish<WTC>(X + xl.p2 + erow[q] * DX_P2 + member * 4 + wave, p2v, tag, rt);
+          const float p2v = fmaxf(s[0][q] + b_p2, 0.f);
+          dx_publish<WTC>(dx_at(X, (unsigned)(xl.p2 + erow[q] * DX_P2 + member * 4 + wave)), p2v, tag, rt);
           if (TAPE && tval[q] && a.tp_p2) a.tp_p2[((size_t)(row0 + erow[q]) * a.n + t) * a.ld_p2 + member * 4 + wave] = p2v;
         }
       }
@@ -875,7 +923,8 @@
     dxq_zero<RG>(ag01);
     dx_zero<1, RG>(ag2);
     dxw_pair<DXR_AGH, RG>(WP, st + DXS_HATT, lane, ag01);
-    dx_gather<RG, DX_P2, false, DXS_LD, DX_NT, DX_DLY(0, DX_POLL_DELAY_B)>(X + xl.p2, tag, st, DXS_P2, 0, 0, tid, rt);
+    dx_ahead<RG>(ag01);
+    dx_gather_at<RG, DX_P2, false, DXS_LD, DX_NT, DX_DLY(0, DX_POLL_DELAY_B)>(X, (unsigned)xl.p2, tag, st, DXS_P2, 0, 0, tid, rt);
     __syncthreads();
     if constexpr (PD == 3) {
       if (wave < 2) {
@@ -886,10 +935,10 @@
         if (epl) {
 #pragma unroll
           for (int q = 0; q < RL; ++q)
-            dx_publish<WTC>(X + xl.p3 + erow[q] * DX_P3 + member * 2 + wave, fmaxf(s[0][q] + bl[DXB_P3 * DX_NW + wave], 0.f), tag, rt);
+            dx_publish<WTC>(dx_at(X, (unsigned)(xl.p3 + erow[q] * DX_P3 + member * 2 + wave)), fmaxf(s[0][q] + bl[DXB_P3 * DX_NW + wave], 0.f), tag, rt);
         }
       }
-      dx_gather<RG, DX_P3, false, DXS_LD, DX_NT, DX_DLY(1, DX_FIRST_POLL_DELAY)>(X + xl.p3, tag, st, DXS_OUT2, 0, 0, tid, rt);
+      dx_gather_at<RG, DX_P3, false, DXS_LD, DX_NT, DX_DLY(1, DX_FIRST_POLL_DELAY)>(X, (unsigned)xl.p3, tag, st, DXS_OUT2, 0, 0, tid, rt);
       __syncthreads();
     }
     DX_STAMP(1);
@@ -906,11 +955,13 @@
         const float rg = dx_sigmoid_fast(s[0][q] + DX_RB(DXRB_AR, q));
         g_u[q] = dx_sigmoid_fast(s[1][q] + DX_RB(DXRB_AU, q));
         g_cx[q] = s[2][q] + DX_RB(DXRB_AX, q);
-        if (epl) dx_publish<WTC>(X + xl.rha + erow[q] * DX_W + en, rg * g_h[q], tag, rt);
+        if (epl) dx_publish<WTC>(dx_at(X, (unsigned)(xl.rha + erow[q] * DX_W + en)), rg * g_h[q], tag, rt);
         DX_TAPE(DXT_RA, q, rg); DX_TAPE(DXT_UA, q, g_u[q]); DX_TAPE(DXT_RHA, q, rg * g_h[q]);
       }
     }
-    dx_gather<RG, DX_W, false, DXS_LD, DX_NT, DX_DLY(2, DX_FIRST_POLL_DELAY)>(X + xl.rha, tag, st, DXS_T, 0, 0, tid, rt);
+    DX_BIAS_AHEAD(b_ac, DXB_AC);
+    dx_gather_at<RG, DX_W, false, DXS_LD, DX_NT, DX_DLY(2, DX_FIRST_POLL_DELAY)>(X, (unsigned)xl.rha, tag, st, DXS_T, 0, 0, tid, rt);
+    DX_BIAS_HERE(b_ac);
     __syncthreads();
     DX_STAMP(2);
     {
@@ -920,15 +971,15 @@
       dxs_reduce<1, RG>(acc, s, lane);
 #pragma unroll
       for (int q = 0; q < RL; ++q) {
-        const float c = taco_tanh_fast(g_cx[q] + s[0][q] + bl[DXB_AC * DX_NW + wave]);
+        const float c = taco_tanh_fast(g_cx[q] + s[0][q] + b_ac);
         const float hn = g_u[q] * g_h[q] + (1.f - g_u[q]) * c;
-        if (epl) dx_publish<WTC>(X + xl.ha + erow[q] * DX_W + en, hn, tag, rt);
+        if (epl) dx_publish<WTC>(dx_at(X, (unsigned)(xl.ha + erow[q] * DX_W + en)), hn, tag, rt);
         DX_TAPE(DXT_CA, q, c); DX_TAPE(DXT_HA, q, hn);
       }
     }
 #pragma unroll
     for (int q = 0; q < RL; ++q) g_h[q] = st[erow[q] * DXS_LD + DXS_H1 + en];
-    dx_gather<RG, DX_W, false, DXS_LD, DX_NT, DX_DLY(3, DX_FIRST_POLL_DELAY)>(X + xl.ha, tag, st, DXS_HATT, 0, 0, tid, rt);
+    dx_gather_at<RG, DX_W, false, DXS_LD, DX_NT, DX_DLY(3, DX_FIRST_POLL_DELAY)>(X, (unsigned)xl.ha, tag, st, DXS_HATT, 0, 0, tid, rt);
     __syncthreads();
     DX_STAMP(3);
     if (!man) {
@@ -978,7 +1029,7 @@
             }
           }
           e = dx_quadsum(e);
-          if (cp == 0 && j < psn) dx_publish<WTC>(X + xl.sc + (size_t)(arow * Pc + cb) * T + ps0 + j, e, tag, rt);
+          if (cp == 0 && j < psn) dx_publish<WTC>(dx_at(X, (unsigned)(xl.sc + (arow * Pc + cb) * T + ps0 + j)), e, tag, rt);
         }
       }
     }
@@ -988,6 +1039,7 @@
     if (G1_AHEAD) {
       dxw_pair<DXR_G1H, RG>(WP, st + DXS_H1, lane, g1p0);
       dxw_quad<DXR_G1A, RG>(WP, st + DXS_HATT, lane, g1p0, g1p1);
+      dx_ahead<RG>(g1p0); dx_ahead<RG>(g1p1);
     }
     int aoff = 0;
     if (!man) {
@@ -998,7 +1050,7 @@
           float s = 0.f;
           if (j < T) {
             float v[NP];
-            dx_poll<NP, DX_DLY(4, DX_POLL_DELAY_B)>(X + xl.sc + (size_t)(arow * Pc + part * NP) * T + j, (size_t)T, tag, v, rt);
+            dx_poll_at<NP, DX_DLY(4, DX_POLL_DELAY_B)>(X, (unsigned)(xl.sc + (arow * Pc + part * NP) * T + j), (unsigned)T, tag, v, rt);
 #pragma unroll
             for (int u = 0; u < NP; ++u) s += v[u];
           }
@@ -1025,12 +1077,6 @@
       aoff = (int)(mrow - sc);
     }
     {
-      for (int j = tid; j < T; j += DX_NT) alp[j] = sc[aoff + j];
-      const int p0 = asl * TP;
-      if (tid < TP && p0 + tid < T && brow < a.B) {
-        if (a.hist) a.hist[((size_t)brow * T + p0 + tid) * a.n + t] = sc[aoff + p0 + tid];
-        if (TAPE && a.tp_alpha) a.tp_alpha[((size_t)brow * (a.n + 1) + t + 1) * T + p0 + tid] = sc[aoff + p0 + tid];
-      }
       constexpr int JL = 64 / DC;
       const int d = lane % DC, jsub = lane / DC;
       float part = 0.f;
@@ -1045,10 +1091,18 @@
       float s = 0.f;
 #pragma unroll
       for (int w = 0; w < DX_NW; ++w) s += cpart[w * 64 + tid];
-      dx_publish<WTC>(X + xl.ctx + arow * DX_W + asl * DC + tid, s, tag, rt);
+      dx_publish<WTC>(dx_at(X, (unsigned)(xl.ctx + arow * DX_W + asl * DC + tid)), s, tag, rt);
       if (TAPE && a.tp_ctx && brow < a.B) a.tp_ctx[((size_t)brow * a.n + t) * a.ld_ctx + asl * DC + tid] = s;
     }
-    dx_gather<RG, DX_W, false, DXS_LD, DX_NT, DX_DLY(5, DX_FIRST_POLL_DELAY)>(X + xl.ctx, tag, st, DXS_CTX, 0, 0, tid, rt);
+    {
+      for (int j = tid; j < T; j += DX_NT) alp[j] = sc[aoff + j];
+      const int p0 = asl * TP;
+      if (tid < TP && p0 + tid < T && brow < a.B) {
+        if (a.hist) a.hist[((size_t)brow * T + p0 + tid) * a.n + t] = sc[aoff + p0 + tid];
+        if (TAPE && a.tp_alpha) a.tp_alpha[((size_t)brow * (a.n + 1) + t + 1) * T + p0 + tid] = sc[aoff + p0 + tid];
+      }
+    }
+    dx_gather_at<RG, DX_W, false, DXS_LD, DX_NT, DX_DLY(5, DX_FIRST_POLL_DELAY)>(X, (unsigned)xl.ctx, tag, st, DXS_CTX, 0, 0, tid, rt);
     __syncthreads();
     DX_STAMP(6);
     {
@@ -1070,12 +1124,14 @@
         g_u[q] = dx_sigmoid_fast(s[1][q] + DX_RB(DXRB_G1U, q));
         g_cx[q] = s[2][q] + DX_RB(DXRB_G1X, q);
         g_o0[q] = s[3][q] + DX_RB(DXRB_O0, q);
-        if (epl) dx_publish<WTC>(X + xl.rh1 + erow[q] * DX_W + en, rg * g_h[q], tag, rt);
+        if (epl) dx_publish<WTC>(dx_at(X, (unsigned)(xl.rh1 + erow[q] * DX_W + en)), rg * g_h[q], tag, rt);
         DX_TAPE(DXT_R1, q, rg); DX_TAPE(DXT_U1, q, g_u[q]); DX_TAPE(DXT_RH1, q, rg * g_h[q]); DX_TAPE(DXT_O0, q, g_o0[q]);
       }
       DX_STAMP(13);
     }
-    dx_gather<RG, DX_W, false, DXS_LD, DX_NT, DX_DLY(6, DX_FIRST_POLL_DELAY)>(X + xl.rh1, tag, st, DXS_T, 0, 0, tid, rt);
+    DX_BIAS_AHEAD(b_g1c, DXB_G1C);
+    dx_gather_at<RG, DX_W, false, DXS_LD, DX_NT, DX_DLY(6, DX_FIRST_POLL_DELAY)>(X, (unsigned)xl.rh1, tag, st, DXS_T, 0, 0, tid, rt);
+    DX_BIAS_HERE(b_g1c);
     DX_STAMP(14);
     __syncthreads();
     DX_STAMP(7);
@@ -1086,12 +1142,12 @@
       dxs_reduce<1, RG>(acc, s, lane);
 #pragma unroll
       for (int q = 0; q < RL; ++q) {
-        const float c = taco_tanh_fast(g_cx[q] + s[0][q] + bl[DXB_G1C * DX_NW + wave]);
+        const float c = taco_tanh_fast(g_cx[q] + s[0][q] + b_g1c);
         const float hn = g_u[q] * g_h[q] + (1.f - g_u[q]) * c;
         g_o1[q] = hn + g_o0[q];
         if (epl) {
-          dx_publish<WTC>(X + xl.h1 + erow[q] * DX_W + en, hn, tag, rt);
-          dx_publish<WTC>(X + xl.o1 + erow[q] * DX_W + en, hn + g_o0[q], tag, rt);
+          dx_publish<WTC>(dx_at(X, (unsigned)(xl.h1 + erow[q] * DX_W + en)), hn, tag, rt);
+          dx_publish<WTC>(dx_at(X, (unsigned)(xl.o1 + erow[q] * DX_W + en)), hn + g_o0[q], tag, rt);
         }
         DX_TAPE(DXT_C1, q, c); DX_TAPE(DXT_H1, q, hn); DX_TAPE(DXT_O1, q, g_o1[q]);
       }
@@ -1102,9 +1158,9 @@
     float g2c[1][RG];
     dxq_zero<RG>(g2p);
     dx_zero<1, RG>(g2c);
-    if (G1_AHEAD) dxw_pair<DXR_G2H, RG>(WP, st + DXS_H2, lane, g2p);
-    dx_gather<RG, DX_W, false, DXS_LD, DX_NT, DX_DLY(7, DX_POLL_DELAY_B)>(X + xl.h1, tag, st, DXS_H1, 0, 0, tid, rt);
-    dx_gather<RG, DX_W, false, DXS_LD, DX_NT, 0>(X + xl.o1, tag, st, DXS_OUT1, 0, 0, tid, rt);
+    if (G1_AHEAD) { dxw_pair<DXR_G2H, RG>(WP, st + DXS_H2, lane, g2p); dx_ahead<RG>(g2p); }
+    dx_gather_at<RG, DX_W, false, DXS_LD, DX_NT, DX_DLY(7, DX_POLL_DELAY_B)>(X, (unsigned)xl.h1, tag, st, DXS_H1, 0, 0, tid, rt);
+    dx_gather_at<RG, DX_W, false, DXS_LD, DX_NT, 0>(X, (unsigned)xl.o1, tag, st, DXS_OUT1, 0, 0, tid, rt);
     __syncthreads();
     DX_STAMP(8);
     {
@@ -1120,11 +1176,13 @@
         const float rg = dx_sigmoid_fast(s[0][q] + bl[DXB_G2R * DX_NW + wave]);
         g_u[q] = dx_sigmoid_fast(s[1][q] + bl[DXB_G2U * DX_NW + wave]);
         g_cx[q] = s[2][q];
-        if (epl) dx_publish<WTC>(X + xl.rh2 + erow[q] * DX_W + en, rg * g_h[q], tag, rt);
+        if (epl) dx_publish<WTC>(dx_at(X, (unsigned)(xl.rh2 + erow[q] * DX_W + en)), rg * g_h[q], tag, rt);
         DX_TAPE(DXT_R2, q, rg); DX_TAPE(DXT_U2, q, g_u[q]); DX_TAPE(DXT_RH2, q, rg * g_h[q]);
       }
     }
-    dx_gather<RG, DX_W, false, DXS_LD, DX_NT, DX_DLY(8, DX_FIRST_POLL_DELAY)>(X + xl.rh2, tag, st, DXS_T, 0, 0, tid, rt);
+    DX_BIAS_AHEAD(b_g2c, DXB_G2C);
+    dx_gather_at<RG, DX_W, false, DXS_LD, DX_NT, DX_DLY(8, DX_FIRST_POLL_DELAY)>(X, (unsigned)xl.rh2, tag, st, DXS_T, 0, 0, tid, rt);
+    DX_BIAS_HERE(b_g2c);
     __syncthreads();
     DX_STAMP(9);
     {
@@ -1134,16 +1192,18 @@
       dxs_reduce<1, RG>(acc, s, lane);
 #pragma unroll
       for (int q = 0; q < RL; ++q) {
-        const float c = taco_tanh_fast(g_cx[q] + s[0][q] + bl[DXB_G2C * DX_NW + wave]);
+        const float c = taco_tanh_fast(g_cx[q] + s[0][q] + b_g2c);
         const float hn = g_u[q] * g_h[q] + (1.f - g_u[q]) * c;
-        if (epl) dx_publish<WTC>(X + xl.h2 + erow[q] * DX_W + en, hn, tag, rt);
+        if (epl) dx_publish<WTC>(dx_at(X, (unsigned)(xl.h2 + erow[q] * DX_W + en)), hn, tag, rt);
         DX_TAPE(DXT_C2, q, c); DX_TAPE(DXT_H2, q, hn); DX_TAPE(DXT_O2, q, hn + g_o1[q]);
       }
     }
     float p1a[1][RG];
     dx_zero<1, RG>(p1a);
-    if (G1_AHEAD) dxw_single<DXR_P1C, RG>(WP, st + DXS_CTX, lane, p1a);
-    dx_gather<RG, DX_W, true, DXS_LD, DX_NT, DX_DLY(9, DX_POLL_DELAY_B)>(X + xl.h2, tag, st, DXS_H2, DXS_OUT1, DXS_OUT2, tid, rt);
+    if (G1_AHEAD) { dxw_single<DXR_P1C, RG>(WP, st + DXS_CTX, lane, p1a); dx_ahead<RG>(p1a); }
+    DX_BIAS_AHEAD(b_p1, DXB_P1); DX_BIAS_AHEAD(b_f0, DXB_F0); DX_BIAS_AHEAD(b_f1, DXB_F1);
+    dx_gather_at<RG, DX_W, true, DXS_LD, DX_NT, DX_DLY(9, DX_POLL_DELAY_B)>(X, (unsigned)xl.h2, tag, st, DXS_H2, DXS_OUT1, DXS_OUT2, tid, rt);
+    DX_BIAS_HERE(b_p1); DX_BIAS_HERE(b_f0); DX_BIAS_HERE(b_f1);
     __syncthreads();
     DX_STAMP(10);
     auto store_frame = [&](int q, float y0, float y1, bool share) {
@@ -1159,8 +1219,8 @@
       }
       if (share) {
         const int f0 = a.rM - a.mels;
-        if (v0 && n0 >= f0) dx_publish<WTC>(X + xl.fb + erow[q] * DX_P2 + (n0 - f0), y0, tag, rt);
-        if (v1 && n1 >= f0) dx_publish<WTC>(X + xl.fb + erow[q] * DX_P2 + (n1 - f0), y1, tag, rt);
+        if (v0 && n0 >= f0) dx_publish<WTC>(dx_at(X, (unsigned)(xl.fb + erow[q] * DX_P2 + (n0 - f0))), y0, tag, rt);
+        if (v1 && n1 >= f0) dx_publish<WTC>(dx_at(X, (unsigned)(xl.fb + erow[q] * DX_P2 + (n1 - f0))), y1, tag, rt);
       }
     };
     if (TAPE && a.own_fb) {
@@ -1181,7 +1241,7 @@
         for (int i = tid; i < RG * a.mels; i += DX_NT) {
           const int r = i / a.mels, j = i - r * a.mels;
           float v[1];
-          dx_poll<1>(X + xl.fb + r * DX_P2 + j, 0, tag, v, rt);
+          dx_poll_at<1>(X, (unsigned)(xl.fb + r * DX_P2 + j), 0u, tag, v, rt);
           tfb[r * DX_W + j] = v[0];
         }
       }
@@ -1197,7 +1257,7 @@
 #pragma unroll
           for (int q = 0; q < RL; ++q) {
             const float p1v = fmaxf(s[0][q] + bl[DXB_P1 * DX_NW + wave], 0.f);
-            dx_publish<WTC>(X + xl.p1 + erow[q] * DX_W + en, p1v, tag, rt);
+            dx_publish<WTC>(dx_at(X, (unsigned)(xl.p1 + erow[q] * DX_W + en)), p1v, tag, rt);
             if (tval[q]) a.tape[(unsigned)DXT_P1 * tstr + trow[q] + (unsigned)(t + 1) * DX_W] = p1v;
           }
         }
@@ -1218,11 +1278,11 @@
 #pragma unroll
         for (int q = 0; q < RL; ++q) {
           if (t + 1 < a.n) {
-            const float p1v = fmaxf(s[2][q] + bl[DXB_P1 * DX_NW + wave], 0.f);
-            dx_publish<WTC>(X + xl.p1 + erow[q] * DX_W + en, p1v, tag, rt);
+            const float p1v = fmaxf(s[2][q] + b_p1, 0.f);
+            dx_publish<WTC>(dx_at(X, (unsigned)(xl.p1 + erow[q] * DX_W + en)), p1v, tag, rt);
             if (TAPE && tval[q]) a.tape[(unsigned)DXT_P1 * tstr + trow[q] + (unsigned)(t + 1) * DX_W] = p1v;
           }
-          store_frame(q, s[0][q] + bl[DXB_F0 * DX_NW + wave], s[1][q] + bl[DXB_F1 * DX_NW + wave], false);
+          store_frame(q, s[0][q] + b_f0, s[1][q] + b_f1, false);
         }
       }
     }
@@ -1233,7 +1293,7 @@
         if (b < a.B) a.dbg[((size_t)t * a.B + b) * a.dbgw + q * DX_W + nn] = st[r * DXS_LD + off + nn];
       }
     }
-    if (t + 1 < a.n) dx_gather<RG, DX_W, false, DXS_LD, DX_NT, DX_DLY(10, DX_FIRST_POLL_DELAY)>(X + xl.p1, tag, st, DXS_T, 0, 0, tid, rt);
+    if (t + 1 < a.n) dx_gather_at<RG, DX_W, false, DXS_LD, DX_NT, DX_DLY(10, DX_FIRST_POLL_DELAY)>(X, (unsigned)xl.p1, tag, st, DXS_T, 0, 0, tid, rt);
     __syncthreads();
     DX_STAMP(11);
   }
```

After: 6.349 million (median of 6 runs). 2.7% higher.
